# Khrylx/EgoPose

Measured on AMD Instinct MI355X. Metric: env-steps/sec (whole node) ego_mimic PPO, higher is better.
Workload: dtype f64 (rollout kernels K1-K6, physics state) + f32 (policy/value nets)

## Files before the change

egopose_amd/_lib.py:

```python
from __future__ import annotations

import ctypes as C
import os

HERE = os.path.dirname(os.path.abspath(__file__))
LIB_PATH = os.path.join(HERE, "libegopose_hip.so")

EGP_OK = 0
EGP_EXPERT_ROW = 168

c_int_p = C.POINTER(C.c_int32)
c_dbl_p = C.POINTER(C.c_double)
vp = C.c_void_p


class ModelDesc(C.Structure):
    _fields_ = [
        ("nq", C.c_int32), ("nv", C.c_int32), ("nu", C.c_int32), ("nbody", C.c_int32), ("nM", C.c_int32),
        ("body_qpos_start", c_int_p), ("body_ndof", c_int_p), ("dof_parentid", c_int_p), ("dof_Madr", c_int_p),
        ("ee_body", c_int_p),
        ("jkp", c_dbl_p), ("jkd", c_dbl_p), ("a_ref", c_dbl_p), ("a_scale", c_dbl_p), ("torque_lim", c_dbl_p),
        ("b_diffw", c_dbl_p),
        ("sub_dt", C.c_double), ("frame_skip", C.c_int32), ("episode_len", C.c_int32),
        ("w_p", C.c_double), ("w_v", C.c_double), ("w_e", C.c_double), ("w_rp", C.c_double), ("w_rv", C.c_double),
        ("k_p", C.c_double), ("k_v", C.c_double), ("k_e", C.c_double), ("k_rh", C.c_double), ("k_rq", C.c_double),
        ("k_rl", C.c_double), ("k_ra", C.c_double),
        ("v_ord", C.c_double), ("decay", C.c_int32),
        ("obs_heading", C.c_int32), ("obs_keep_root_heading", C.c_int32), ("obs_coord_root", C.c_int32), ("obs_vel", C.c_int32),
        ("action_torque", C.c_int32), ("obs_phase", C.c_int32),
    ]


class ExpertTable(C.Structure):
    _fields_ = [
        ("n_takes", C.c_int32), ("n_frames", C.c_int32), ("take_offset", c_int_p),
        ("qpos", c_dbl_p), ("qvel", c_dbl_p), ("rlinv_local", c_dbl_p), ("rangv", c_dbl_p), ("rq_rmh", c_dbl_p),
        ("ee_pos", c_dbl_p), ("bquat", c_dbl_p), ("bangvel", c_dbl_p), ("head_height_lb", c_dbl_p),
    ]


class SurrogateDesc(C.Structure):
    _fields_ = [
        ("nq", C.c_int32), ("nv", C.c_int32), ("nu", C.c_int32), ("nbody", C.c_int32), ("nM", C.c_int32),
        ("njoint", C.c_int32),
        ("qM0", c_dbl_p), ("Minv0", c_dbl_p), ("body_parent", c_int_p), ("body_pos", c_dbl_p), ("body_ndof", c_int_p),
        ("joint_axis", c_dbl_p), ("joint_anchor", c_dbl_p),
        ("sub_dt", C.c_double), ("damping", C.c_double), ("support_k", C.c_double), ("support_c", C.c_double),
    ]


class DynamicsDesc(C.Structure):
    _fields_ = [("nbody", C.c_int32), ("njoint", C.c_int32), ("body_parent", c_int_p), ("body_pos", c_dbl_p), ("body_com", c_dbl_p),
                ("body_inertia", c_dbl_p), ("body_mass", c_dbl_p), ("body_ndof", c_int_p), ("joint_axis", c_dbl_p),
                ("joint_anchor", c_dbl_p), ("armature", C.c_double), ("gravity", C.c_double * 3)]


class MlpLayer(C.Structure):
    _fields_ = [("wt", vp), ("bias", vp), ("in_dim", C.c_int32), ("out_dim", C.c_int32)]


class GemmDesc(C.Structure):
    _fields_ = [("M", C.c_int32), ("N", C.c_int32), ("K", C.c_int32),
                ("A", vp), ("lda", C.c_int64), ("a_kcontig", C.c_int32),
                ("B", vp), ("ldb", C.c_int64), ("b_kcontig", C.c_int32),
                ("C", vp), ("ldc", C.c_int64),
                ("bias", vp), ("relu", C.c_int32),
                ("mask", vp), ("ldmask", C.c_int64),
                ("terms", C.c_int32), ("splits", C.c_int32), ("accumulate", C.c_int32),
                ("bias_grad", vp), ("workspace", vp),
                ("a_rows", vp), ("A2", vp), ("lda2", C.c_int64), ("a_split", C.c_int32), ("a_src_rows", C.c_int64),
                ("b_krows", vp), ("B2", vp), ("ldb2", C.c_int64), ("b_split", C.c_int32), ("b_src_rows", C.c_int64),
                ("c_rows", vp), ("a_krows", vp)]


class PpoLossDesc(C.Structure):
    _fields_ = [("n", C.c_int32), ("n_pol", C.c_int32), ("act_dim", C.c_int32),
                ("rows", vp), ("pred", vp), ("returns", vp),
                ("mean", vp), ("ld_mean", C.c_int64),
                ("actions", vp), ("ld_act", C.c_int64),
                ("log_std", vp), ("adv", vp),
                ("fixed_logp", vp), ("write_fixed", C.c_int32),
                ("clip_eps", C.c_double), ("inv_n_val", C.c_double), ("inv_n_exp", C.c_double),
                ("d_pred", vp), ("d_mean", vp), ("ld_dmean", C.c_int64), ("d_log_std", vp),
                ("losses", vp), ("workspace", vp)]


class MinibatchPlanDesc(C.Structure):
    _fields_ = [("n", C.c_int32), ("state_dim", C.c_int32), ("act_dim", C.c_int32), ("batch", C.c_int32),
                ("perm", vp),
                ("states", vp), ("ld_states", C.c_int64),
                ("actions", vp), ("ld_act", C.c_int64),
                ("returns", vp), ("adv", vp), ("fixed_logp", vp), ("exps", vp),
                ("out_states", vp), ("out_actions", vp), ("out_returns", vp), ("out_adv", vp), ("out_fixed_logp", vp), ("out_exps", vp),
                ("mb_n_exp", vp)]


class PpoLossMbDesc(C.Structure):
    _fields_ = [("n", C.c_int32), ("act_dim", C.c_int32),
                ("pred", vp), ("returns", vp),
                ("mean", vp), ("ld_mean", C.c_int64),
                ("actions", vp), ("ld_act", C.c_int64),
                ("log_std", vp),
                ("adv", vp), ("fixed_logp", vp), ("exps", vp),
                ("n_exp", vp),
                ("clip_eps", C.c_double),
                ("d_pred", vp),
                ("d_mean", vp), ("ld_dmean", C.c_int64),
                ("d_log_std", vp),
                ("losses", vp)]


PPO_LOSS_MB_MAX_ROWS = 16384


class TcnDesc(C.Structure):
    _fields_ = [("T", C.c_int32), ("B", C.c_int32), ("C_in", C.c_int32), ("C_out", C.c_int32),
                ("taps", C.c_int32), ("shift0", C.c_int32), ("dshift", C.c_int32),
                ("X", vp), ("ldx", C.c_int64),
                ("W", vp),
                ("bias", vp), ("relu", C.c_int32),
                ("mask", vp), ("ldmask", C.c_int64),
                ("gate", vp), ("ldgate", C.c_int64),
                ("X2", vp), ("ldx2", C.c_int64), ("C2", C.c_int32), ("W2", vp), ("b2", vp), ("x2_after_act", C.c_int32),
                ("out", vp), ("ldout", C.c_int64),
                ("out2", vp), ("ldout2", C.c_int64)]


class AdamSegment(C.Structure):
    _fields_ = [("begin", C.c_int64), ("end", C.c_int64),
                ("lr", C.c_double), ("beta1", C.c_double), ("beta2", C.c_double), ("eps", C.c_double), ("weight_decay", C.c_double),
                ("bias1", C.c_double), ("bias2", C.c_double), ("max_norm", C.c_double),
                ("clip_group", C.c_int32)]


ADAM_MAX_SEGMENTS = 8


class RolloutTick(C.Structure):
    _fields_ = [("ctx", vp), ("eng", vp), ("stream", vp),
                ("n_env", C.c_int32), ("nmax", C.c_int32), ("obs_dim", C.c_int32), ("nu", C.c_int32), ("nq", C.c_int32), ("nv", C.c_int32),
                ("ctx_dim", C.c_int32), ("ctx_T", C.c_int32), ("episode_len", C.c_int32), ("reward_job", C.c_int32),
                ("has_fix_head_lb", C.c_int32),
                ("end_reward", C.c_double), ("zf_clip", C.c_double), ("fix_head_lb", C.c_double),
                ("cur_t", vp), ("frame_base", vp), ("e_ind", vp), ("s_ind", vp), ("steps_done", vp),
                ("active", vp), ("active_i32", vp), ("head_z", vp), ("head_lb", vp),
                ("rec_valid", vp), ("rec_done", vp), ("rec_e_ind", vp), ("rec_s_ind", vp),
                ("states", vp), ("next_states", vp), ("actions", vp), ("rewards", vp), ("cinfo", vp),
                ("noise", vp), ("v_out", vp), ("v_stride", C.c_int64),
                ("layers", vp), ("n_layers", C.c_int32), ("activation", C.c_int32), ("log_std", vp),
                ("slab_host", vp), ("slab_dev", vp),
                ("qpos", vp), ("qvel", vp), ("prev_qpos", vp), ("ee", vp),
                ("zf_workspace", vp), ("reset_scratch", vp),
                ("defer_apply", C.c_int32)]


class HostProbeResult(C.Structure):
    _fields_ = [(k, C.c_double) for k in ("pcie_read_gbps", "pcie_read_us_per_pass", "go_rtt_us_p50", "go_rtt_us_p99", "go_rtt_us_max",
                                          "spin_gap_us_max", "spin_gap_us_median_of_thread_max", "spin_lost_frac")] + \
               [(k, C.c_int32) for k in ("pcie_read_rows", "go_rtt_n", "go_in_vram", "large_bar", "spin_threads", "spin_gaps_over_5us")]


class EngineDesc(C.Structure):
    _fields_ = [("n_env", C.c_int32), ("n_threads", C.c_int32), ("n_groups", C.c_int32), ("device_dynamics", C.c_int32)]


PHYS_RESET = C.CFUNCTYPE(C.c_int, vp, C.c_int32, c_dbl_p, c_dbl_p)
PHYS_STEP = C.CFUNCTYPE(C.c_int, vp, C.c_int32, c_dbl_p)
PHYS_DRAIN = C.CFUNCTYPE(C.c_int, vp, C.c_int32, c_dbl_p, c_dbl_p, c_dbl_p, c_dbl_p, c_dbl_p)
PHYS_DESTROY = C.CFUNCTYPE(None, vp)
PHYS_EPOCH = C.CFUNCTYPE(C.c_int64, vp, C.c_int32)


class PhysicsVtable(C.Structure):
    _fields_ = [("user", vp), ("reset", PHYS_RESET), ("step", PHYS_STEP), ("drain", PHYS_DRAIN),
                ("destroy", PHYS_DESTROY), ("name", C.c_char_p), ("inertia_epoch", PHYS_EPOCH)]


_i32, _i64, _f64 = C.c_int32, C.c_int64, C.c_double
SIGNATURES = {
    "egp_last_error": (C.c_char_p, []),
    "egp_version": (C.c_char_p, []),
    "egp_abi_sizeof": (C.c_int64, [C.c_char_p]),
    "egp_obs_dim": (_i32, [vp]),
    "egp_create": (C.c_int, [C.POINTER(ModelDesc), C.c_int, C.POINTER(vp)]),
    "egp_destroy": (C.c_int, [vp]),
    "egp_set_reward_weights": (C.c_int, [vp, C.POINTER(ModelDesc)]),
    "egp_set_pd_variant": (C.c_int, [vp, C.c_int]),
    "egp_upload_experts": (C.c_int, [vp, C.POINTER(ExpertTable)]),
    "egp_reward_simple_f64": (C.c_int, [vp, _i32, vp, vp, vp, vp, C.c_double, _i32, vp, vp, vp]),
    "egp_quat_op_f64": (C.c_int, [_i32, vp, vp, _i32, vp, vp]),
    "egp_quat_op_f32": (C.c_int, [_i32, vp, vp, _i32, vp, vp]),
    "egp_body_quat_f64": (C.c_int, [vp, vp, _i32, vp, vp]),
    "egp_body_quat_f32": (C.c_int, [vp, vp, _i32, vp, vp]),
    "egp_obs_f64": (C.c_int, [vp, vp, vp, vp, _i32, vp, vp]),
    "egp_obs_f32": (C.c_int, [vp, vp, vp, vp, _i32, vp, vp]),
    "egp_pd_torque_f64": (C.c_int, [vp, vp, vp, vp, vp, vp, _i32, vp, vp, vp]),
    "egp_pd_torque_f32": (C.c_int, [vp, vp, vp, vp, vp, vp, _i32, vp, vp, vp]),
    "egp_reward_quat_v3_f64": (C.c_int, [vp, vp, vp, vp, vp, vp, vp, vp, _f64, _i32, vp, vp, vp]),
    "egp_reward_quat_v3_f32": (C.c_int, [vp, vp, vp, vp, vp, vp, vp, vp, _f64, _i32, vp, vp, vp]),
    "egp_pose_features_f64": (C.c_int, [vp, vp, vp, vp, _i32, _i32, vp, vp, vp, vp, vp, vp, vp, vp]),
    "egp_pose_features_f32": (C.c_int, [vp, vp, vp, vp, _i32, _i32, vp, vp, vp, vp, vp, vp, vp, vp]),
    "egp_zfilter_workspace_bytes": (_i64, [_i32, _i32]),
    "egp_zfilter_f64": (C.c_int, [vp, vp, _i32, _i32, vp, vp, _i32, _f64, vp, vp, vp]),
    "egp_zfilter_f32": (C.c_int, [vp, vp, _i32, _i32, vp, vp, _i32, _f64, vp, vp, vp]),
    "egp_obs_zfilter_f64": (C.c_int, [vp, vp, vp, vp, vp, _i32, vp, vp, _f64, vp, vp, _i32, vp, vp]),
    "egp_obs_zfilter_f32": (C.c_int, [vp, vp, vp, vp, vp, _i32, vp, vp, _f64, vp, vp, _i32, vp, vp]),
    "egp_gae_workspace_bytes": (_i64, [_i32]),
    "egp_gae_f64": (C.c_int, [vp, vp, vp, _i32, _f64, _f64, vp, vp, vp, vp, vp]),
    "egp_gae_f32": (C.c_int, [vp, vp, vp, _i32, _f64, _f64, vp, vp, vp, vp, vp]),
    "egp_gae_standardize_f64": (C.c_int, [vp, _i32, vp, vp]),
    "egp_gae_standardize_f32": (C.c_int, [vp, _i32, vp, vp]),
    "egp_lstm_gate_layout": (_i32, []),
    "egp_gather_concat_f32": (C.c_int, [vp, _i64, vp, vp, _i64, _i32, _i32, _i32, vp, _i64, vp]),
    "egp_scatter_rows_f32": (C.c_int, [vp, _i64, vp, _i32, _i32, vp, _i64, vp]),
    "egp_gemm_workspace_floats": (_i64, [_i32, _i32, _i32, _i32]),
    "egp_gemm_f32": (C.c_int, [C.POINTER(GemmDesc), vp]),
    "egp_ppo_loss_workspace_bytes": (_i64, [_i32, _i32, _i32]),
    "egp_ppo_loss_f32": (C.c_int, [C.POINTER(PpoLossDesc), vp]),
    "egp_minibatch_plan_f32": (C.c_int, [C.POINTER(MinibatchPlanDesc), vp]),
    "egp_ppo_loss_mb_f32": (C.c_int, [C.POINTER(PpoLossMbDesc), vp]),
    "egp_tcn_conv_f32": (C.c_int, [C.POINTER(TcnDesc), vp]),
    "egp_adam_workspace_bytes": (_i64, []),
    "egp_adam_step_f32": (C.c_int, [_i32, C.POINTER(AdamSegment), vp, vp, vp, vp, vp, vp, vp]),
    "egp_adam_step_f64": (C.c_int, [_i32, C.POINTER(AdamSegment), vp, vp, vp, vp, vp, vp, vp, vp]),
    "egp_adam_step_f64g": (C.c_int, [_i32, C.POINTER(AdamSegment), vp, vp, vp, vp, vp, vp, vp]),
    "egp_lstm_fwd_f32": (C.c_int, [vp, vp, _i32, _i32, _i32, _i32, vp, vp, vp, vp]),
    "egp_lstm_bwd_f32": (C.c_int, [vp, vp, vp, vp, _i32, _i32, _i32, _i32, vp, vp]),
    "egp_lstm_group_fwd_f32": (C.c_int, [vp, vp, _i32, _i32, _i32, _i32, _i32, C.POINTER(C.c_void_p), _i32, vp, vp, vp]),
    "egp_lstm_group_bwd_f32": (C.c_int, [C.POINTER(C.c_void_p), _i32, vp, vp, vp, _i32, _i32, _i32, _i32, _i32, vp, vp, vp]),
    "egp_rollout_tick_pre": (C.c_int, [vp, _i32, _i32, _i32, _i32, vp, _i32, vp, vp]),
    "egp_rollout_tick_apply": (C.c_int, [vp, _i32, _i32, _i32, _i32, vp, vp]),
    "egp_obs_zfilter_split_max_rows": (C.c_int32, []),
    "egp_obs_zfilter_stats_f64": (C.c_int, [vp, vp, vp, vp, vp, _i32, vp, vp]),
    "egp_obs_zfilter_apply_f64": (C.c_int, [vp, vp, vp, vp, _i32, vp, vp, C.c_double, vp, vp, vp, vp]),
    "egp_policy_gaussian_filter_f32": (C.c_int, [vp, vp, C.c_int64, _i32, vp, vp, vp, vp, _i32, vp, vp, C.c_double, vp, vp, vp,
                                                vp, _i32, _i32, vp, vp, vp, vp, vp, vp, C.c_int64, vp]),
    "egp_rollout_tick_post": (C.c_int, [vp, _i32, _i32, _i32, _i32, vp, vp, vp, vp]),
    "egp_rollout_reset": (C.c_int, [vp, _i32, _i32, _i32, _i32, vp, _i32, vp, vp, vp, vp, vp, vp, vp, vp, vp]),
    "egp_engine_group_stream": (vp, [vp, _i32]),
    "egp_debug_burn": (C.c_int, [C.c_int64, _i32, vp, vp]),
    "egp_lstm_group_fwd_len_f32": (C.c_int, [vp, vp, _i32, _i32, _i32, _i32, _i32, C.POINTER(C.c_void_p), _i32, vp, vp, vp, vp, _i32, vp, vp]),
    "egp_lstm_group_bwd_len_f32": (C.c_int, [C.POINTER(C.c_void_p), _i32, vp, vp, vp, _i32, _i32, _i32, _i32, _i32, vp, vp, vp, vp, _i32, vp]),
    "egp_lstm_group_bwd_rows_f32": (C.c_int, [C.POINTER(C.c_void_p), _i32, vp, vp, vp, _i32, _i32, _i32, _i32, _i32, vp, vp, vp, vp, _i32, vp]),
    "egp_set_dynamics_model": (C.c_int, [vp, C.POINTER(DynamicsDesc)]),
    "egp_dynamics_f64": (C.c_int, [vp, vp, vp, _i32, vp, C.c_int64, vp, vp, vp]),
    "egp_set_pose2d_bodies": (C.c_int, [vp, c_int_p, c_int_p]),
    "egp_pose2d_f64": (C.c_int, [vp, vp, vp, vp, vp, vp, vp, C.c_int64, vp]),
    "egp_mlp_pack_floats": (C.c_int64, [_i32, _i32]),
    "egp_mlp_pack_f32": (C.c_int, [vp, C.c_int64, _i32, _i32, vp, vp]),
    "egp_policy_gaussian_f32": (C.c_int, [vp, C.c_int64, _i32, vp, vp, _i32, _i32, C.POINTER(MlpLayer), _i32, _i32, vp, vp, vp, vp, vp]),
    "egp_policy_forecast_f32": (C.c_int, [vp, C.c_int64, _i32, vp, vp, _i32, C.POINTER(MlpLayer), vp, vp, C.c_int64, _i32,
                                          C.POINTER(MlpLayer), _i32, _i32, vp, vp, vp, vp, vp]),
    "egp_policy_forecast_filter_f32": (C.c_int, [vp, vp, C.c_int64, _i32, vp, vp, vp, vp, _i32, vp, vp, C.c_double, vp, vp, vp,
                                                 C.POINTER(MlpLayer), vp, vp, C.c_int64, C.POINTER(MlpLayer), _i32, _i32, vp, vp, vp, vp, vp]),
    "egp_policy_value_filter_f32": (C.c_int, [vp, vp, C.c_int64, _i32, vp, C.c_int64, _i32, vp, vp, vp, vp, _i32, vp, vp, C.c_double, vp, vp,
                                              C.POINTER(MlpLayer), _i32, _i32, vp, vp, vp, vp, C.POINTER(MlpLayer), _i32, _i32, vp, vp]),
    "egp_policy_gaussian_staged_f32": (C.c_int, [vp, C.c_int64, _i32, vp, vp, _i32, _i32, C.POINTER(MlpLayer), _i32, _i32, vp, vp, vp, vp, vp, vp,
                                                 C.c_int64, vp]),
    "egp_physics_register": (C.c_int, [C.POINTER(PhysicsVtable), _i32, C.POINTER(vp)]),
    "egp_physics_create_surrogate": (C.c_int, [C.POINTER(SurrogateDesc), _i32, C.POINTER(vp)]),
    "egp_physics_destroy": (C.c_int, [vp]),
    "egp_physics_name": (C.c_char_p, [vp]),
    "egp_physics_n_env": (_i32, [vp]),
    "egp_physics_reset_host": (C.c_int, [vp, _i32, vp, vp]),
    "egp_physics_step_host": (C.c_int, [vp, _i32, vp]),
    "egp_physics_drain_host": (C.c_int, [vp, _i32, vp, vp, vp, vp, vp]),
    "egp_engine_create": (C.c_int, [vp, vp, C.POINTER(EngineDesc), C.POINTER(vp)]),
    "egp_engine_destroy": (C.c_int, [vp]),
    "egp_engine_state": (C.c_int, [vp] + [C.POINTER(vp)] * 7),
    "egp_engine_reset": (C.c_int, [vp, vp, _i32, vp, vp, vp]),
    "egp_engine_step_async": (C.c_int, [vp, _i32, vp, vp, vp]),
    "egp_engine_wait": (C.c_int, [vp, _i32, vp]),
    "egp_engine_timing": (C.c_int, [vp, c_dbl_p, c_dbl_p, c_dbl_p, C.POINTER(_i64)]),
    "egp_engine_reset_timing": (C.c_int, [vp]),
    "egp_engine_inertia_uploads": (_i64, [vp]),
    "egp_engine_k1_env_substeps": (_i64, [vp]),
    "egp_engine_event_overhead_ms": (C.c_double, [vp]),
    "egp_engine_set_profile": (C.c_int, [vp, C.c_int]),
    "egp_engine_layout": (C.c_int, [vp, c_int_p, c_int_p, c_int_p, c_int_p]),
    "egp_engine_group_range": (C.c_int, [vp, _i32, c_int_p, c_int_p]),
    "egp_engine_set_reward_job": (C.c_int, [vp, _i32, vp, vp, vp, vp, _f64, vp, vp]),
    "egp_engine_substeps_per_launch": (C.c_int, [vp]),
    "egp_engine_server_trace": (C.c_int, [vp, _i32, vp, vp]),
    "egp_engine_go_words_in_vram": (_i32, [vp]),
    "egp_engine_envs_per_wave": (_i32, [vp, C.POINTER(C.c_int32)]),
    "egp_host_probe": (C.c_int, [_i32, _i32, _i32, C.POINTER(HostProbeResult)]),
    "egp_device_usable_cus": (_i32, [_i32]),
}

_lib = None


class EgpError(RuntimeError):
    pass


def load():
    global _lib
    if _lib is not None:
        return _lib
    if not os.path.exists(LIB_PATH):
        raise EgpError(
            "egopose_amd: %s is missing -- build it with `python -m egopose_amd.build` "
            "(hipcc --offload-arch=gfx950). There is no CPU fallback for the product path." % LIB_PATH)
    lib = C.CDLL(LIB_PATH, mode=C.RTLD_GLOBAL)
    for name, (res, args) in SIGNATURES.items():
        try:
            fn = getattr(lib, name)
        except AttributeError as e:
            raise EgpError("egopose_amd: symbol %s not exported by %s" % (name, LIB_PATH)) from e
        fn.restype = res
        fn.argtypes = args
    _lib = lib
    return lib


def check(rc, what=""):
    if rc == EGP_OK:
        return
    msg = load().egp_last_error().decode("utf-8", "replace")
    text = "%s failed (%d): %s" % (what or "egp call", rc, msg)
    if rc == -1:
        raise ValueError(text)
    raise EgpError(text)


def current_stream(device_index=None):
    import torch
    try:
        if device_index is None:
            device_index = torch._C._cuda_getDevice()
        return C.c_void_p(torch._C._cuda_getCurrentRawStream(device_index))
    except AttributeError:
        return C.c_void_p(torch.cuda.current_stream(device_index).cuda_stream)
```

egopose_amd/csrc/egp_lstm.hip:

```cpp
#include <hip/hip_runtime.h>
#include <math.h>
#include <stdlib.h>

#include "egp_internal.hpp"

namespace egp {

constexpr int KC = 64;

__device__ __forceinline__ float sigmoidf_(float x) { return __builtin_amdgcn_rcpf(1.0f + __expf(-x)); }
__device__ __forceinline__ float tanhf_(float x) { return 2.0f * __builtin_amdgcn_rcpf(1.0f + __expf(-2.0f * x)) - 1.0f; }

typedef float f32x4 __attribute__((ext_vector_type(4)));

#ifndef EGP_LSTM_NT
#define EGP_LSTM_NT 3
#endif
template <typename V> __device__ __forceinline__ void st_save(V *p, V v) {
    if constexpr ((EGP_LSTM_NT & 1) != 0) __builtin_nontemporal_store(v, p); else *p = v;
}
template <typename V> __device__ __forceinline__ V ld_save(const V *p) {
    if constexpr ((EGP_LSTM_NT & 1) != 0) return __builtin_nontemporal_load(p); else return *p;
}
template <typename V> __device__ __forceinline__ void st_dpre(V *p, V v) {
    if constexpr ((EGP_LSTM_NT & 2) != 0) __builtin_nontemporal_store(v, p); else *p = v;
}

struct LstmGroup {
    int ld_g;
    int rev_mask;
    int ld_h;
    int ld_dh;
    long c_stride;
    float *h[4];
    const float *dh[4];
    float *db;
    int db_rows;
    const int *order;
    const int *steps;
    int leave_skipped;
    const int *seq_base;
};

template <int ROWS>
__device__ __forceinline__ int lstm_group_steps(const LstmGroup &grp, int reverse, int r0, int B, int T) {
    if (reverse || !grp.steps) return T;
    int mx = 0;
#pragma unroll
    for (int i = 0; i < ROWS; ++i)
        if (r0 + i < B) mx = max(mx, grp.steps[r0 + i]);
    return min(T, mx);
}

#ifdef EGP_LSTM_TRACE
__device__ long long g_lstm_trace[8];
#define EGP_LT_DECL long long lt_acc[6] = {0, 0, 0, 0, 0, 0}, lt_prev = 0; const bool lt_on = blockIdx.x == EGP_LSTM_TRACE && blockIdx.y == 0 && threadIdx.x == 0
#define EGP_LT_START if (lt_on) lt_prev = (long long)__builtin_readcyclecounter()
#define EGP_LT(i) if (lt_on) { const long long lt_now = (long long)__builtin_readcyclecounter(); lt_acc[i] += lt_now - lt_prev; lt_prev = lt_now; }
#define EGP_LT_END(steps) if (lt_on) { for (int i = 0; i < 6; ++i) g_lstm_trace[i] = lt_acc[i]; g_lstm_trace[6] = (steps); }
#else
#define EGP_LT_DECL do { } while (0)
#define EGP_LT_START do { } while (0)
#define EGP_LT(i) do { } while (0)
#define EGP_LT_END(steps) do { } while (0)
#endif
#ifndef EGP_LSTM_PD1
#define EGP_LSTM_PD1 (NQ == 1 ? 4 : 4)
#endif
#ifndef EGP_LSTM_KCH
#define EGP_LSTM_KCH (NQ == 1 && LH == 64 ? 32 : 64)
#endif
#ifndef EGP_LSTM_BPD
#define EGP_LSTM_BPD ((NQ == 1 && LH == 64) ? 4 : 2)
#endif
#ifndef EGP_LSTM_BKCH
#define EGP_LSTM_BKCH 64
#endif
template <int NQ, int LH, bool FULL, bool TRAIN>
__global__ __launch_bounds__(4 * LH) void k_lstm_fwd_mfma(const float *__restrict__ gx, const float *__restrict__ w_hh, int T, int B,
                                                          LstmGroup grp, float *__restrict__ gates_out, float *__restrict__ c_out) {
    constexpr int LG = 4 * LH, ROWS = 4 * NQ;
    const int prob = (int)(gridDim.y - 1 - blockIdx.y), reverse = (grp.rev_mask >> prob) & 1, ld = grp.ld_g, ld_h = grp.ld_h;
    float *__restrict__ h_out = grp.h[prob];
    gx += prob * LG; w_hh += (long)prob * LG * LH;
    if (TRAIN) { gates_out += prob * LG; c_out += prob * grp.c_stride; }
    constexpr int PD = LH == 128 ? 2 : EGP_LSTM_PD1;
    __shared__ __attribute__((aligned(16))) float s_h[2][ROWS][LH + 4];
    const int lane = threadIdx.x & 63, wave = threadIdx.x >> 6;
    const int u = 16 * wave + (lane >> 2), sub = lane & 3;
    const int r0 = blockIdx.x * ROWS;
    float w[LH];
#pragma unroll
    for (int k = 0; k < LH; ++k) w[k] = w_hh[(long)(sub * LH + u) * LH + k];
    float cst[NQ];
    f32x4 pre[PD][NQ];
    bool live[NQ];
    int rowc[NQ];
#pragma unroll
    for (int q = 0; q < NQ; ++q) {
        cst[q] = 0.f;
        live[q] = FULL || r0 + 4 * q + sub < B;
        const int pos = live[q] ? r0 + 4 * q + sub : B - 1;
        rowc[q] = grp.order ? grp.order[pos] : pos;
    }
    const long gmul = grp.seq_base ? 1 : B;
    long gadd[NQ];
#pragma unroll
    for (int q = 0; q < NQ; ++q) gadd[q] = grp.seq_base ? (long)grp.seq_base[rowc[q]] : (long)rowc[q];
    const int Tp = lstm_group_steps<ROWS>(grp, reverse, r0, B, T);
    for (int i = threadIdx.x; i < 2 * ROWS * (LH + 4); i += 4 * LH) (&s_h[0][0][0])[i] = 0.f;

#define EGP_LSTM_FETCH_GX(STEP, DST)                                                                 \
    {                                                                                                \
        const int f_s = (STEP) < T ? (STEP) : T - 1;                                                 \
        const int f_t = reverse ? T - 1 - f_s : f_s;                                                 \
        _Pragma("unroll") for (int q = 0; q < NQ; ++q)                                               \
            DST[q] = *reinterpret_cast<const f32x4 *>(gx + ((long)f_t * gmul + gadd[q]) * ld + 4 * u); \
    }

    EGP_LT_DECL;
    auto do_step = [&](const int step, const int par, const f32x4 (&init)[NQ]) {
        const int t = reverse ? T - 1 - step : step;
        EGP_LT(0);
        f32x4 acc[NQ], acc2[NQ];
#pragma unroll
        for (int q = 0; q < NQ; ++q) { acc[q] = init[q]; acc2[q] = f32x4{0.f, 0.f, 0.f, 0.f}; }
        constexpr int KCH = EGP_LSTM_KCH;
#pragma unroll
        for (int kc = 0; kc < LH; kc += KCH) {
            float4 hv[NQ][KCH / 4];
#pragma unroll
            for (int q = 0; q < NQ; ++q)
#pragma unroll
                for (int k4 = 0; k4 < KCH / 4; ++k4) hv[q][k4] = *reinterpret_cast<const float4 *>(&s_h[par][4 * q + sub][kc + 4 * k4]);
            __builtin_amdgcn_sched_barrier(0);
            EGP_LT(1);
#pragma unroll
            for (int k4 = 0; k4 < KCH / 4; ++k4)
#pragma unroll
                for (int q = 0; q < NQ; ++q) {
                    acc[q] = __builtin_amdgcn_mfma_f32_4x4x1f32(w[kc + 4 * k4 + 0], hv[q][k4].x, acc[q], 0, 0, 0);
                    acc2[q] = __builtin_amdgcn_mfma_f32_4x4x1f32(w[kc + 4 * k4 + 1], hv[q][k4].y, acc2[q], 0, 0, 0);
                    acc[q] = __builtin_amdgcn_mfma_f32_4x4x1f32(w[kc + 4 * k4 + 2], hv[q][k4].z, acc[q], 0, 0, 0);
                    acc2[q] = __builtin_amdgcn_mfma_f32_4x4x1f32(w[kc + 4 * k4 + 3], hv[q][k4].w, acc2[q], 0, 0, 0);
                }
        }
        EGP_LT(2);
#pragma unroll
        for (int q = 0; q < NQ; ++q) {
            const f32x4 a = acc[q] + acc2[q];
            const float ig = sigmoidf_(a[0]), fg = sigmoidf_(a[1]), gg = tanhf_(a[2]), og = sigmoidf_(a[3]);
            const float cn = fg * cst[q] + ig * gg;
            const float hn = og * tanhf_(cn);
            cst[q] = cn;
            s_h[par ^ 1][4 * q + sub][u] = hn;
            if (FULL || live[q]) {
                const long row = (long)t * B + rowc[q];
                h_out[row * ld_h + u] = hn;
                if (TRAIN) {
                    st_save(reinterpret_cast<f32x4 *>(gates_out + row * ld + 4 * u), f32x4{ig, fg, gg, og});
                    st_save(c_out + row * LH + u, cn);
                }
            }
        }
        EGP_LT(3);
        __syncthreads();
        EGP_LT(4);
    };

#pragma unroll
    for (int d = 0; d < PD; ++d) EGP_LSTM_FETCH_GX(d, pre[d])
    __syncthreads();
    EGP_LT_START;
    int s0 = 0;
    for (; s0 + PD <= Tp; s0 += PD) {
        f32x4 cur[PD][NQ];
#pragma unroll
        for (int d = 0; d < PD; ++d)
#pragma unroll
            for (int q = 0; q < NQ; ++q) cur[d][q] = pre[d][q];
#pragma unroll
        for (int d = 0; d < PD; ++d) EGP_LSTM_FETCH_GX(s0 + PD + d, pre[d])
#pragma unroll
        for (int d = 0; d < PD; ++d) do_step(s0 + d, d & 1, cur[d]);
    }
    for (int d = 0; s0 + d < Tp; ++d) {
        f32x4 last[NQ];
#pragma unroll
        for (int q = 0; q < NQ; ++q) last[q] = d == 0 ? pre[0][q] : d == 1 ? pre[1 % PD][q] : d == 2 ? pre[2 % PD][q] : d == 3 ? pre[3 % PD][q]
                                             : d == 4 ? pre[4 % PD][q] : d == 5 ? pre[5 % PD][q] : pre[6 % PD][q];
        do_step(s0 + d, d & 1, last);
    }
#undef EGP_LSTM_FETCH_GX
    EGP_LT_END(Tp);
    const int Tz = grp.leave_skipped ? lstm_group_steps<8>(grp, reverse, r0 & ~7, B, T) : T;
    for (int t = Tp; t < Tz; ++t)
#pragma unroll
        for (int q = 0; q < NQ; ++q)
            if (FULL || live[q]) h_out[((long)t * B + rowc[q]) * ld_h + u] = 0.f;
}

template <int NQ, int LH, bool FULL>
__global__ __launch_bounds__(4 * LH) void k_lstm_bwd_mfma(const float *__restrict__ gates, const float *__restrict__ cells,
                                                          const float *__restrict__ w_hh, int T, int B, LstmGroup grp,
                                                          float *__restrict__ dpre) {
    constexpr int LG = 4 * LH, NT = 4 * LH, ROWS = 4 * NQ, UH = LH / 64;
    const int prob = (int)(gridDim.y - 1 - blockIdx.y), reverse = (grp.rev_mask >> prob) & 1, ld = grp.ld_g, ld_dh = grp.ld_dh;
    const float *__restrict__ dh_out = grp.dh[prob];
    gates += prob * LG; dpre += prob * LG; cells += prob * grp.c_stride; w_hh += (long)prob * LG * LH;
    constexpr int NP = (ROWS * LH + NT - 1) / NT;
    constexpr int PD = EGP_LSTM_BPD;
    __shared__ __attribute__((aligned(16))) float s_d[ROWS][LG + 4];
    __shared__ float s_part[4][ROWS][LH + 1];
    const int lane = threadIdx.x & 63, wave = threadIdx.x >> 6;
    const int q = wave / UH, uh = wave % UH, sub = lane & 3;
    const int r0 = blockIdx.x * ROWS;
    float w[LH];
#pragma unroll
    for (int cc = 0; cc < LH; ++cc) {
        const int n = q * LH + cc;
        w[cc] = w_hh[(long)((n & 3) * LH + (n >> 2)) * LH + 64 * uh + lane];
    }
    float dc_next[NP], dh_rec[NP];
    f32x4 dsum[NP];
    f32x4 pg[PD][NP];
    float pc[PD][NP], pdh[PD][NP];
    bool live[NP];
    int rowc[NP];
#pragma unroll
    for (int qq = 0; qq < NP; ++qq) {
        dc_next[qq] = 0.f; dh_rec[qq] = 0.f; dsum[qq] = f32x4{0.f, 0.f, 0.f, 0.f};
        const int r = (threadIdx.x + NT * qq) / LH;
        live[qq] = FULL || r0 + r < B;
        const int pos = live[qq] ? r0 + r : B - 1;
        rowc[qq] = grp.order ? grp.order[pos] : pos;
    }
    const int Tp = lstm_group_steps<ROWS>(grp, reverse, r0, B, T);
    const int Tz = grp.leave_skipped ? lstm_group_steps<8>(grp, reverse, r0 & ~7, B, T) : T;
    for (int t = Tp; t < Tz; ++t)
#pragma unroll
        for (int qq = 0; qq < NP; ++qq)
            if (FULL || live[qq])
                *reinterpret_cast<f32x4 *>(dpre + ((long)t * B + rowc[qq]) * ld + 4 * ((threadIdx.x + NT * qq) % LH)) = f32x4{0.f, 0.f, 0.f, 0.f};

#define EGP_LSTM_FETCH(STEP, D)                                                                      \
    {                                                                                                \
        const int f_s = (STEP) > 0 ? (STEP) : 0;                                                     \
        const int f_t = reverse ? T - 1 - f_s : f_s;                                                 \
        _Pragma("unroll") for (int qq = 0; qq < NP; ++qq) {                                          \
            const int j = (threadIdx.x + NT * qq) % LH;                                              \
            const long row = (long)f_t * B + rowc[qq];                                               \
            pg[D][qq] = ld_save(reinterpret_cast<const f32x4 *>(gates + row * ld + 4 * j));         \
            pc[D][qq] = ld_save(cells + row * LH + j);                                               \
            pdh[D][qq] = dh_out[row * ld_dh + j];                                                    \
        }                                                                                            \
    }

    auto do_step = [&](const int step, const f32x4 (&g4)[NP], const float (&cc_)[NP], const float (&cdh)[NP], const float (&cprev)[NP]) {
        const int t = reverse ? T - 1 - step : step;
#pragma unroll
        for (int qq = 0; qq < NP; ++qq) {
            const int p = threadIdx.x + NT * qq, r = p / LH, j = p % LH;
            const float ig = g4[qq][0], fg = g4[qq][1], gg = g4[qq][2], og = g4[qq][3];
            const float c_prev = step > 0 ? cprev[qq] : 0.f;
            const float tc = tanhf_(cc_[qq]);
            const float dh = (FULL || live[qq] ? cdh[qq] : 0.f) + dh_rec[qq];
            const float dc = dh * og * (1.f - tc * tc) + dc_next[qq];
            const float d_o = dh * tc * og * (1.f - og);
            const float di = dc * gg * ig * (1.f - ig);
            const float df = dc * c_prev * fg * (1.f - fg);
            const float dg = dc * ig * (1.f - gg * gg);
            dc_next[qq] = dc * fg;
            const f32x4 d4 = f32x4{di, df, dg, d_o};
            if (FULL || live[qq]) { st_dpre(reinterpret_cast<f32x4 *>(dpre + ((long)t * B + rowc[qq]) * ld + 4 * j), d4); dsum[qq] += d4; }
            *reinterpret_cast<f32x4 *>(&s_d[r][4 * j]) = d4;
        }
        __syncthreads();
        f32x4 acc[NQ], acc2[NQ];
#pragma unroll
        for (int qd = 0; qd < NQ; ++qd) acc[qd] = acc2[qd] = f32x4{0.f, 0.f, 0.f, 0.f};
#pragma unroll
        for (int kc = 0; kc < LH; kc += EGP_LSTM_BKCH) {
            float4 dv[NQ][EGP_LSTM_BKCH / 4];
#pragma unroll
            for (int qd = 0; qd < NQ; ++qd)
#pragma unroll
                for (int c4 = 0; c4 < EGP_LSTM_BKCH / 4; ++c4) dv[qd][c4] = *reinterpret_cast<const float4 *>(&s_d[4 * qd + sub][q * LH + kc + 4 * c4]);
            __builtin_amdgcn_sched_barrier(0);
#pragma unroll
            for (int c4 = 0; c4 < EGP_LSTM_BKCH / 4; ++c4)
#pragma unroll
                for (int qd = 0; qd < NQ; ++qd) {
                    acc[qd] = __builtin_amdgcn_mfma_f32_4x4x1f32(w[kc + 4 * c4 + 0], dv[qd][c4].x, acc[qd], 0, 0, 0);
                    acc2[qd] = __builtin_amdgcn_mfma_f32_4x4x1f32(w[kc + 4 * c4 + 1], dv[qd][c4].y, acc2[qd], 0, 0, 0);
                    acc[qd] = __builtin_amdgcn_mfma_f32_4x4x1f32(w[kc + 4 * c4 + 2], dv[qd][c4].z, acc[qd], 0, 0, 0);
                    acc2[qd] = __builtin_amdgcn_mfma_f32_4x4x1f32(w[kc + 4 * c4 + 3], dv[qd][c4].w, acc2[qd], 0, 0, 0);
                }
        }
#pragma unroll
        for (int qd = 0; qd < NQ; ++qd) {
            const f32x4 a = acc[qd] + acc2[qd];
#pragma unroll
            for (int i = 0; i < 4; ++i) s_part[q][4 * qd + sub][64 * uh + (lane & ~3) + i] = a[i];
        }
        __syncthreads();
#pragma unroll
        for (int qq = 0; qq < NP; ++qq) {
            const int p = threadIdx.x + NT * qq, r = p / LH, j = p % LH;
            dh_rec[qq] = s_part[0][r][j] + s_part[1][r][j] + s_part[2][r][j] + s_part[3][r][j];
        }
    };

#pragma unroll
    for (int d = 0; d < PD; ++d) EGP_LSTM_FETCH(Tp - 1 - d, d)
    int s0 = Tp - 1;
    for (; s0 - PD + 1 >= 0; s0 -= PD) {
        f32x4 cg[PD][NP];
        float cc_[PD][NP], cdh[PD][NP];
#pragma unroll
        for (int d = 0; d < PD; ++d)
#pragma unroll
            for (int qq = 0; qq < NP; ++qq) {
                cg[d][qq] = pg[d][qq];
                cc_[d][qq] = pc[d][qq];
                cdh[d][qq] = pdh[d][qq];
            }
#pragma unroll
        for (int d = 0; d < PD; ++d) EGP_LSTM_FETCH(s0 - PD - d, d)
#pragma unroll
        for (int d = 0; d < PD; ++d)
            do_step(s0 - d, cg[d], cc_[d], cdh[d], d + 1 < PD ? cc_[d + 1 < PD ? d + 1 : 0] : pc[0]);
    }
#pragma unroll
    for (int d = 0; d < PD - 1; ++d)
        if (s0 - d >= 0) do_step(s0 - d, pg[d], pc[d], pdh[d], pc[d + 1]);
#undef EGP_LSTM_FETCH
    if (grp.db) {
        __syncthreads();
#pragma unroll
        for (int qq = 0; qq < NP; ++qq) {
            const int p = threadIdx.x + NT * qq;
            *reinterpret_cast<f32x4 *>(&s_d[p / LH][4 * (p % LH)]) = dsum[qq];
        }
        __syncthreads();
        if (grp.db_rows) {
            for (int p = threadIdx.x; p < ROWS * LG; p += NT) {
                const int r = p / LG, c = p % LG;
                if (FULL || r0 + r < B) grp.db[((long)prob * B + r0 + r) * LG + c] = s_d[r][c];
            }
        } else {
            for (int c = threadIdx.x; c < LG; c += NT) {
                float a = 0.f;
#pragma unroll
                for (int r = 0; r < ROWS; ++r) a += s_d[r][c];
                atomicAdd(grp.db + prob * LG + c, a);
            }
        }
    }
}

}

using namespace egp;

static int lstm_quads(int B) { return B >= 4096 ? 2 : 1; }

static int lstm_launch_check(const char *what) {
    hipError_t e = hipGetLastError();
    if (e != hipSuccess) {
        set_error("launch of %s failed: %s", what, hipGetErrorString(e));
        return EGP_E_HIP;
    }
    return EGP_OK;
}

template <int NQ, int LH>
static void launch_fwd_mfma_t(bool full, bool train, int P, const float *gx, const float *w_hh, int T, int B, const LstmGroup &g,
                              float *gates_save, float *cells_save, hipStream_t s) {
    const dim3 grid((B + 4 * NQ - 1) / (4 * NQ), P), block(4 * LH);
    if (full && train) k_lstm_fwd_mfma<NQ, LH, true, true><<<grid, block, 0, s>>>(gx, w_hh, T, B, g, gates_save, cells_save);
    else if (full) k_lstm_fwd_mfma<NQ, LH, true, false><<<grid, block, 0, s>>>(gx, w_hh, T, B, g, gates_save, cells_save);
    else if (train) k_lstm_fwd_mfma<NQ, LH, false, true><<<grid, block, 0, s>>>(gx, w_hh, T, B, g, gates_save, cells_save);
    else k_lstm_fwd_mfma<NQ, LH, false, false><<<grid, block, 0, s>>>(gx, w_hh, T, B, g, gates_save, cells_save);
}
static void launch_fwd_mfma(int hidden, int P, const float *gx, const float *w_hh, int T, int B, const LstmGroup &g,
                            float *gates_save, float *cells_save, hipStream_t s) {
    const int nq = hidden == 64 ? lstm_quads(B) : 1;
    const bool full = B % (4 * nq) == 0, train = gates_save != nullptr;
    if (hidden == 128) launch_fwd_mfma_t<1, 128>(full, train, P, gx, w_hh, T, B, g, gates_save, cells_save, s);
    else if (nq >= 2) launch_fwd_mfma_t<2, 64>(full, train, P, gx, w_hh, T, B, g, gates_save, cells_save, s);
    else launch_fwd_mfma_t<1, 64>(full, train, P, gx, w_hh, T, B, g, gates_save, cells_save, s);
}

template <int NQ, int LH>
static void launch_bwd_mfma_t(bool full, int P, const float *gates_save, const float *cells_save, const float *w_hh, int T, int B,
                              const LstmGroup &g, float *d_pre, hipStream_t s) {
    const dim3 grid((B + 4 * NQ - 1) / (4 * NQ), P), block(4 * LH);
    if (full) k_lstm_bwd_mfma<NQ, LH, true><<<grid, block, 0, s>>>(gates_save, cells_save, w_hh, T, B, g, d_pre);
    else k_lstm_bwd_mfma<NQ, LH, false><<<grid, block, 0, s>>>(gates_save, cells_save, w_hh, T, B, g, d_pre);
}
static void launch_bwd_mfma(int hidden, int P, const float *gates_save, const float *cells_save, const float *w_hh, int T, int B,
                            const LstmGroup &g, float *d_pre, hipStream_t s) {
    const int nq = hidden == 64 ? lstm_quads(B) : 1;
    const bool full = B % (4 * nq) == 0;
    if (hidden == 128) launch_bwd_mfma_t<1, 128>(full, P, gates_save, cells_save, w_hh, T, B, g, d_pre, s);
    else if (nq >= 2) launch_bwd_mfma_t<2, 64>(full, P, gates_save, cells_save, w_hh, T, B, g, d_pre, s);
    else launch_bwd_mfma_t<1, 64>(full, P, gates_save, cells_save, w_hh, T, B, g, d_pre, s);
}

static int lstm_group_bwd(const float *const *dh_out, int32_t ld_dh, const float *gates_save, const float *cells_save, const float *w_hh,
                          int32_t T, int32_t B, int32_t hidden, int32_t n_problems, int32_t reverse_mask, float *d_pre, float *d_bias,
                          int db_rows, const int32_t *seq_order, const int32_t *seq_steps, int32_t leave_skipped, void *stream) {
    EGP_REQUIRE((seq_order == nullptr) == (seq_steps == nullptr), "seq_order and seq_steps go together");
    EGP_REQUIRE(hidden == 64 || hidden == 128, "egp_lstm kernels are built for hidden size 64 and 128");
    EGP_REQUIRE(n_problems >= 1 && n_problems <= 4, "1..4 problems per group");
    EGP_REQUIRE(T >= 0 && B >= 0, "negative size");
    if (T == 0 || B == 0) return EGP_OK;
    EGP_REQUIRE(dh_out && gates_save && cells_save && w_hh && d_pre && ld_dh >= hidden, "NULL pointer / d h_out row stride below the hidden size");
    LstmGroup g = {};
    g.ld_g = 4 * hidden * n_problems; g.rev_mask = reverse_mask; g.ld_dh = ld_dh; g.c_stride = (long)T * B * hidden; g.db = d_bias; g.db_rows = db_rows;
    for (int p = 0; p < n_problems; ++p) {
        EGP_REQUIRE(dh_out[p], "NULL d h_out");
        g.dh[p] = dh_out[p];
    }
    g.order = seq_order; g.steps = seq_steps; g.leave_skipped = seq_steps && leave_skipped;
    launch_bwd_mfma(hidden, n_problems, gates_save, cells_save, w_hh, T, B, g, d_pre, (hipStream_t)stream);
    return lstm_launch_check("k_lstm_bwd_mfma (group)");
}

extern "C" {

int32_t egp_lstm_gate_layout(void) { return EGP_LSTM_GATES_UNIT_MAJOR; }

int egp_lstm_fwd_f32(const float *gates_x, const float *w_hh, int32_t T, int32_t B, int32_t hidden, int32_t reverse,
                     float *h_out, float *gates_save, float *cells_save, void *stream) {
    EGP_REQUIRE(hidden == 64 || hidden == 128, "egp_lstm kernels are built for hidden size 64 and 128");
    EGP_REQUIRE(T >= 0 && B >= 0, "negative size");
    if (T == 0 || B == 0) return EGP_OK;
    EGP_REQUIRE(gates_x && w_hh && h_out, "NULL pointer");
    EGP_REQUIRE((gates_save == nullptr) == (cells_save == nullptr), "gates_save and cells_save go together");
    hipStream_t s = (hipStream_t)stream;
    LstmGroup g = {};
    g.ld_g = 4 * hidden; g.rev_mask = reverse ? 1 : 0; g.ld_h = hidden; g.h[0] = h_out;
    launch_fwd_mfma(hidden, 1, gates_x, w_hh, T, B, g, gates_save, cells_save, s);
    return lstm_launch_check("k_lstm_fwd");
}

int egp_lstm_bwd_f32(const float *dh_out, const float *gates_save, const float *cells_save, const float *w_hh, int32_t T, int32_t B,
                     int32_t hidden, int32_t reverse, float *d_pre, void *stream) {
    EGP_REQUIRE(hidden == 64 || hidden == 128, "egp_lstm kernels are built for hidden size 64 and 128");
    EGP_REQUIRE(T >= 0 && B >= 0, "negative size");
    if (T == 0 || B == 0) return EGP_OK;
    EGP_REQUIRE(dh_out && gates_save && cells_save && w_hh && d_pre, "NULL pointer");
    hipStream_t s = (hipStream_t)stream;
    LstmGroup g = {};
    g.ld_g = 4 * hidden; g.rev_mask = reverse ? 1 : 0; g.ld_dh = hidden; g.dh[0] = dh_out;
    launch_bwd_mfma(hidden, 1, gates_save, cells_save, w_hh, T, B, g, d_pre, s);
    return lstm_launch_check("k_lstm_bwd");
}

int egp_lstm_group_fwd_f32(const float *gates_x, const float *w_hh, int32_t T, int32_t B, int32_t hidden, int32_t n_problems,
                           int32_t reverse_mask, float *const *h_out, int32_t ld_h, float *gates_save, float *cells_save, void *stream) {
    return egp_lstm_group_fwd_len_f32(gates_x, w_hh, T, B, hidden, n_problems, reverse_mask, h_out, ld_h, gates_save, cells_save, nullptr, nullptr, 0,
                                      nullptr, stream);
}

int egp_lstm_group_fwd_len_f32(const float *gates_x, const float *w_hh, int32_t T, int32_t B, int32_t hidden, int32_t n_problems,
                               int32_t reverse_mask, float *const *h_out, int32_t ld_h, float *gates_save, float *cells_save,
                               const int32_t *seq_order, const int32_t *seq_steps, int32_t leave_skipped, const int32_t *seq_base,
                               void *stream) {
    EGP_REQUIRE((seq_order == nullptr) == (seq_steps == nullptr), "seq_order and seq_steps go together");
    EGP_REQUIRE(!seq_base || !gates_save || gates_save != gates_x, "a frame table cannot double as the saved gates (rows are shared between sequences)");
    EGP_REQUIRE(hidden == 64 || hidden == 128, "egp_lstm kernels are built for hidden size 64 and 128");
    EGP_REQUIRE(n_problems >= 1 && n_problems <= 4, "1..4 problems per group");
    EGP_REQUIRE(T >= 0 && B >= 0, "negative size");
    if (T == 0 || B == 0) return EGP_OK;
    EGP_REQUIRE(gates_x && w_hh && h_out && ld_h >= hidden, "NULL pointer / h_out row stride below the hidden size");
    EGP_REQUIRE((gates_save == nullptr) == (cells_save == nullptr), "gates_save and cells_save go together");
    LstmGroup g = {};
    g.ld_g = 4 * hidden * n_problems; g.rev_mask = reverse_mask; g.ld_h = ld_h; g.c_stride = (long)T * B * hidden;
    for (int p = 0; p < n_problems; ++p) {
        EGP_REQUIRE(h_out[p], "NULL h_out");
        g.h[p] = h_out[p];
    }
    g.order = seq_order; g.steps = seq_steps; g.leave_skipped = seq_steps && leave_skipped; g.seq_base = seq_base;
    launch_fwd_mfma(hidden, n_problems, gates_x, w_hh, T, B, g, gates_save, cells_save, (hipStream_t)stream);
    return lstm_launch_check("k_lstm_fwd_mfma (group)");
}

int egp_lstm_group_bwd_f32(const float *const *dh_out, int32_t ld_dh, const float *gates_save, const float *cells_save, const float *w_hh,
                           int32_t T, int32_t B, int32_t hidden, int32_t n_problems, int32_t reverse_mask, float *d_pre, float *d_bias,
                           void *stream) {
    return egp_lstm_group_bwd_len_f32(dh_out, ld_dh, gates_save, cells_save, w_hh, T, B, hidden, n_problems, reverse_mask, d_pre, d_bias, nullptr,
                                      nullptr, 0, stream);
}

int egp_lstm_group_bwd_len_f32(const float *const *dh_out, int32_t ld_dh, const float *gates_save, const float *cells_save, const float *w_hh,
                               int32_t T, int32_t B, int32_t hidden, int32_t n_problems, int32_t reverse_mask, float *d_pre, float *d_bias,
                               const int32_t *seq_order, const int32_t *seq_steps, int32_t leave_skipped, void *stream) {
    return lstm_group_bwd(dh_out, ld_dh, gates_save, cells_save, w_hh, T, B, hidden, n_problems, reverse_mask, d_pre, d_bias, 0, seq_order,
                          seq_steps, leave_skipped, stream);
}

int egp_lstm_group_bwd_rows_f32(const float *const *dh_out, int32_t ld_dh, const float *gates_save, const float *cells_save, const float *w_hh,
                                int32_t T, int32_t B, int32_t hidden, int32_t n_problems, int32_t reverse_mask, float *d_pre, float *d_bias_rows,
                                const int32_t *seq_order, const int32_t *seq_steps, int32_t leave_skipped, void *stream) {
    EGP_REQUIRE(d_bias_rows, "NULL d_bias_rows");
    if (T == 0 && B > 0 && n_problems >= 1 && n_problems <= 4) {
        EGP_HIP_CHECK(hipMemsetAsync(d_bias_rows, 0, sizeof(float) * (size_t)n_problems * B * 4 * hidden, (hipStream_t)stream));
        return EGP_OK;
    }
    return lstm_group_bwd(dh_out, ld_dh, gates_save, cells_save, w_hh, T, B, hidden, n_problems, reverse_mask, d_pre, d_bias_rows, 1, seq_order,
                          seq_steps, leave_skipped, stream);
}

}
```

egopose_amd/gemm.py:

```python
from __future__ import annotations

import ctypes as C
import os

import torch

from . import _lib as L

_WS = {}


def enabled():
    return os.environ.get("EGP_GEMM", "hip") != "torch"


def default_terms():
    t = os.environ.get("EGP_GEMM_TERMS", "6")
    if t not in ("1", "3", "6"):
        raise ValueError("EGP_GEMM_TERMS must be 1, 3 or 6, got %r" % t)
    return int(t)


_WS_MAX = 8


def _workspace(n_floats, device):
    key = (str(device), int(torch.cuda.current_stream(device).cuda_stream))
    buf = _WS.pop(key, None)
    if buf is None or buf.numel() < n_floats:
        buf = torch.empty(max(int(n_floats), 1 << 20), dtype=torch.float32, device=device)
    _WS[key] = buf
    while len(_WS) > _WS_MAX:
        _WS.pop(next(iter(_WS)))
    return buf


def _mat(t, name):
    if not (t.is_cuda and t.dtype == torch.float32 and t.dim() == 2):
        raise ValueError("%s must be a 2-D float32 HIP tensor, got %s %s" % (name, tuple(t.shape), t.dtype))
    if t.shape[1] > 1 and t.stride(1) != 1:
        raise ValueError("%s must have unit stride along its second dimension (strides %s)" % (name, t.stride()))
    return t


def _ld(t):
    return t.stride(0) if t.shape[0] > 1 else max(t.shape[1], 1)


_CUS = {}


def usable_cus(device=None):
    if not torch.cuda.is_available():
        return 256
    dev = torch.cuda.current_device() if device is None else int(device)
    if dev not in _CUS:
        n = int(L.load().egp_device_usable_cus(dev))
        _CUS[dev] = n if n > 0 else 256
    return _CUS[dev]


def pick_splits(M, n_out, K):
    cus = usable_cus()
    if M == 1:
        return max(1, min(cus, K // 128))
    tiles = ((M + 127) // 128) * ((n_out + 127) // 128)
    return max(1, min(cus // tiles, K // 256))


def _index(t, name):
    if not (t.is_cuda and t.dtype == torch.int64 and t.dim() == 1 and t.is_contiguous()):
        raise ValueError("%s must be a contiguous 1-D int64 HIP tensor" % name)
    return t


def gemm(A, B, a_kcontig=True, b_kcontig=True, bias=None, relu=False, mask=None, terms=None, splits=1, want_bias_grad=False,
         out=None, bias_grad_out=None, accumulate=False, a_rows=None, a2=None, b_krows=None, b2=None, c_rows=None, a_krows=None):
    A, B = _mat(A, "A"), _mat(B, "B")
    if accumulate and not (splits > 1 or want_bias_grad):
        raise ValueError("accumulate goes with splits > 1 or want_bias_grad (a plain product overwrites `out`)")
    M, K = (A.shape if a_kcontig else A.shape[::-1])
    N, Kb = (B.shape if b_kcontig else B.shape[::-1])
    a_split = b_split = 0
    if a_rows is not None or a2 is not None:
        if not a_kcontig:
            raise ValueError("a_rows / a2 go with a k-contiguous A")
        if a_rows is not None:
            M = _index(a_rows, "a_rows").shape[0]
        if a2 is not None:
            _mat(a2, "a2")
            if a2.shape[0] != M:
                raise ValueError("a2 has %d rows, the operand %d" % (a2.shape[0], M))
            a_split, K = K, K + a2.shape[1]
    if a_krows is not None:
        if a_kcontig:
            raise ValueError("a_krows goes with A given as (K, M)")
        K = _index(a_krows, "a_krows").shape[0]
    if b_krows is not None or b2 is not None:
        if b_kcontig:
            raise ValueError("b_krows / b2 go with B given as (K, N)")
        if b_krows is not None:
            Kb = _index(b_krows, "b_krows").shape[0]
        if b2 is not None:
            _mat(b2, "b2")
            if b2.shape[0] != Kb:
                raise ValueError("b2 has %d rows, the operand %d" % (b2.shape[0], Kb))
            b_split, N = N, N + b2.shape[1]
    if K != Kb:
        raise ValueError("inner dimensions differ: %d vs %d" % (K, Kb))
    dev = A.device
    if c_rows is not None:
        if out is None or _index(c_rows, "c_rows").shape[0] != M:
            raise ValueError("c_rows needs `out` (the scatter destination) and one entry per result row")
    elif out is None:
        out = torch.empty(M, N, dtype=torch.float32, device=dev)
    _mat(out, "out")
    d = L.GemmDesc()
    d.M, d.N, d.K = M, N, K
    if a_rows is not None:
        d.a_rows, d.a_src_rows = a_rows.data_ptr(), A.shape[0]
    if a2 is not None:
        d.A2, d.lda2, d.a_split = a2.data_ptr(), _ld(a2), a_split
    if b_krows is not None:
        d.b_krows, d.b_src_rows = b_krows.data_ptr(), B.shape[0]
    if b2 is not None:
        d.B2, d.ldb2, d.b_split = b2.data_ptr(), _ld(b2), b_split
    if c_rows is not None:
        d.c_rows = c_rows.data_ptr()
    if a_krows is not None:
        d.a_krows = a_krows.data_ptr()
    d.A, d.lda, d.a_kcontig = A.data_ptr(), _ld(A), 1 if a_kcontig else 0
    d.B, d.ldb, d.b_kcontig = B.data_ptr(), _ld(B), 1 if b_kcontig else 0
    d.C, d.ldc = out.data_ptr(), _ld(out)
    d.bias = bias.data_ptr() if bias is not None else None
    d.relu = 1 if relu else 0
    if mask is not None:
        _mat(mask, "mask")
        d.mask, d.ldmask = mask.data_ptr(), _ld(mask)
    d.terms = int(terms or default_terms())
    d.splits = int(splits)
    d.accumulate = 1 if accumulate else 0
    bg = None
    if want_bias_grad:
        bg = bias_grad_out if bias_grad_out is not None else torch.empty(M, dtype=torch.float32, device=dev)
        d.bias_grad = bg.data_ptr()
    if splits > 1 or want_bias_grad:
        ws = _workspace(L.load().egp_gemm_workspace_floats(M, N, 1 if want_bias_grad else 0, int(splits)), dev)
        d.workspace = ws.data_ptr()
    L.check(L.load().egp_gemm_f32(C.byref(d), L.current_stream()), "egp_gemm_f32")
    return (out, bg) if want_bias_grad else out


def linear_fwd(x, W, b=None, relu=False, terms=None):
    return gemm(x, W, True, True, bias=b, relu=relu, terms=terms)


def linear_dgrad(dy, W, mask=None, n_cols=None, terms=None):
    Wv = W if n_cols is None else W[:, :n_cols]
    return gemm(dy, Wv, True, False, mask=mask, terms=terms)


def linear_wgrad(dy, x, want_bias=True, terms=None):
    K, M = dy.shape
    n_out = x.shape[1] + (1 if want_bias else 0)
    return gemm(dy, x, False, False, terms=terms, splits=pick_splits(M, n_out, K), want_bias_grad=want_bias)


class MlpHead(torch.autograd.Function):

    @staticmethod
    def forward(ctx, x, n_grad_cols, *params):
        Ws, bs = params[0::2], params[1::2]
        hs = [x.contiguous()]
        for i, (W, b) in enumerate(zip(Ws, bs)):
            hs.append(linear_fwd(hs[-1], W.contiguous(), b, relu=i < len(Ws) - 1))
        ctx.save_for_backward(*hs[:-1], *Ws)
        ctx.n_layers, ctx.n_grad_cols = len(Ws), int(n_grad_cols)
        return hs[-1]

    @staticmethod
    def backward(ctx, dout):
        nl = ctx.n_layers
        hs, Ws = ctx.saved_tensors[:nl], ctx.saved_tensors[nl:]
        dz = dout.contiguous()
        grads = [None] * (2 * nl)
        dx = None
        for i in range(nl - 1, -1, -1):
            need_w, need_b = ctx.needs_input_grad[2 + 2 * i], ctx.needs_input_grad[3 + 2 * i]
            if need_w or need_b:
                dW, db = linear_wgrad(dz, hs[i], want_bias=True)
                grads[2 * i], grads[2 * i + 1] = (dW if need_w else None), (db if need_b else None)
            if i > 0:
                dz = linear_dgrad(dz, Ws[i].contiguous(), mask=hs[i])
            elif ctx.needs_input_grad[0]:
                nc = ctx.n_grad_cols
                W0 = Ws[0].contiguous()
                if nc >= W0.shape[1]:
                    dx = linear_dgrad(dz, W0)
                else:
                    dx = torch.zeros(dz.shape[0], W0.shape[1], dtype=dz.dtype, device=dz.device)
                    gemm(dz, W0[:, :nc], True, False, out=dx[:, :nc])
        return (dx, None, *grads)


def mlp_head_available(x, layers, head, activation):
    if isinstance(x, GatheredInput):
        x = x.x
    if not (enabled() and x.is_cuda and x.dtype == torch.float32 and x.dim() == 2 and activation is torch.relu):
        return False
    return all(l.weight.dtype == torch.float32 and l.bias is not None and l.weight.is_cuda for l in list(layers) + [head])


def mlp_head(x, layers, head, n_grad_cols=None):
    params = []
    for l in list(layers) + [head]:
        params += [l.weight, l.bias]
    nc = x.shape[1] if n_grad_cols is None else int(n_grad_cols)
    return MlpHead.apply(x, nc, *params)


class GatheredInput:

    def __init__(self, ctx2d, idx, x):
        self.ctx2d, self.idx, self.x = ctx2d, idx, x
        self.shape = (x.shape[0], ctx2d.shape[1] + x.shape[1])
        self.dtype, self.device, self.is_cuda = x.dtype, x.device, x.is_cuda

    def dim(self):
        return 2

    def size(self, k=None):
        return torch.Size(self.shape) if k is None else self.shape[k]

    def materialize(self):
        return GatherConcat.apply(self.ctx2d, self.idx, self.x)

    def __getitem__(self, ind):
        if torch.is_tensor(ind) and ind.dtype == torch.int64 and ind.dim() == 1:
            return GatheredInput(self.ctx2d, self.idx.index_select(0, ind), self.x.index_select(0, ind))
        return self.materialize()[ind]


def fused_gather_available(H, n_hidden, S):
    import os
    return enabled() and default_terms() == 6 and os.environ.get("EGP_GEMM_WS", "1") != "0" and H % 128 == 0 and n_hidden % 4 == 0 \
        and S >= 32


def fused_rows_available():
    import os
    return enabled() and default_terms() == 6 and os.environ.get("EGP_GEMM_WS", "1") != "0"


class GatherMlpHead(torch.autograd.Function):

    @staticmethod
    def forward(ctx, ctx2d, idx, x, *params):
        Ws, bs = params[0::2], params[1::2]
        ctx2d, x = ctx2d.contiguous(), (x if x.stride(1) == 1 else x.contiguous())
        h = gemm(ctx2d, Ws[0].contiguous(), True, True, bias=bs[0], relu=len(Ws) > 1, a_rows=idx, a2=x)
        hs = [h]
        for i in range(1, len(Ws)):
            hs.append(linear_fwd(hs[-1], Ws[i].contiguous(), bs[i], relu=i < len(Ws) - 1))
        ctx.save_for_backward(ctx2d, idx, x, *hs[:-1], *Ws)
        ctx.n_layers = len(Ws)
        return hs[-1]

    @staticmethod
    def backward(ctx, dout):
        nl = ctx.n_layers
        ctx2d, idx, x = ctx.saved_tensors[:3]
        hs, Ws = ctx.saved_tensors[3:3 + nl - 1], ctx.saved_tensors[3 + nl - 1:]
        dz = dout.contiguous()
        grads = [None] * (2 * nl)
        for i in range(nl - 1, 0, -1):
            need_w, need_b = ctx.needs_input_grad[3 + 2 * i], ctx.needs_input_grad[4 + 2 * i]
            if need_w or need_b:
                dW, db = linear_wgrad(dz, hs[i - 1], want_bias=True)
                grads[2 * i], grads[2 * i + 1] = (dW if need_w else None), (db if need_b else None)
            dz = linear_dgrad(dz, Ws[i].contiguous(), mask=hs[i - 1])
        H, S = ctx2d.shape[1], x.shape[1]
        if ctx.needs_input_grad[3] or ctx.needs_input_grad[4]:
            n = dz.shape[0]
            dW, db = gemm(dz, ctx2d, False, False, splits=pick_splits(dz.shape[1], H + S + 1, n), want_bias_grad=True, b_krows=idx, b2=x)
            grads[0], grads[1] = (dW if ctx.needs_input_grad[3] else None), (db if ctx.needs_input_grad[4] else None)
        dctx = None
        if ctx.needs_input_grad[0]:
            dctx = torch.zeros_like(ctx2d)
            gemm(dz, Ws[0][:, :H], True, False, out=dctx, c_rows=idx)
        return (dctx, None, None, *grads)


def gather_mlp_head(gi, layers, head):
    params = []
    for l in list(layers) + [head]:
        params += [l.weight, l.bias]
    return GatherMlpHead.apply(gi.ctx2d, gi.idx, gi.x, *params)


class GatherConcat(torch.autograd.Function):

    @staticmethod
    def forward(ctx, ctx2d, idx, x):
        n, H, S = idx.shape[0], ctx2d.shape[1], x.shape[1]
        out = torch.empty(n, H + S, dtype=torch.float32, device=x.device)
        L.check(L.load().egp_gather_concat_f32(ctx2d.data_ptr(), _ld(ctx2d), idx.data_ptr(), x.data_ptr(), _ld(x), n, H, S,
                                               out.data_ptr(), H + S, L.current_stream()), "egp_gather_concat_f32")
        ctx.save_for_backward(idx)
        ctx.shape = tuple(ctx2d.shape)
        return out

    @staticmethod
    def backward(ctx, dout):
        (idx,) = ctx.saved_tensors
        if not ctx.needs_input_grad[0]:
            return None, None, None
        R, H = ctx.shape
        dout = _mat(dout if dout.stride(1) == 1 else dout.contiguous(), "dout")
        dctx = torch.zeros(R, H, dtype=torch.float32, device=dout.device)
        L.check(L.load().egp_scatter_rows_f32(dout.data_ptr(), _ld(dout), idx.data_ptr(), idx.shape[0], H, dctx.data_ptr(), H,
                                              L.current_stream()), "egp_scatter_rows_f32")
        return dctx, None, None


def gather_concat_available(ctx2d, idx, x):
    return (enabled() and x.is_cuda and ctx2d.dtype == torch.float32 and x.dtype == torch.float32 and ctx2d.dim() == 2 and x.dim() == 2
            and ctx2d.is_contiguous() and x.stride(1) == 1 and idx.dtype == torch.int64 and idx.is_contiguous() and not x.requires_grad)
```

egopose_amd/lstm.py:

```python
from __future__ import annotations

import ctypes as C
import os

import numpy as np
import torch

from . import _lib as L
from . import gemm as G

HIDDEN_SIZES = (64, 128)


def available(x, cell):
    return (x.is_cuda and x.dtype == torch.float32 and cell.hidden_size in HIDDEN_SIZES
            and cell.weight_hh.dtype == torch.float32 and cell.bias_ih is not None)


def _s():
    return L.current_stream()


def _p(t):
    return C.c_void_p(t.data_ptr()) if t is not None else C.c_void_p(0)


_PERM = {}


def _gate_perm(hidden, device):
    if L.load().egp_lstm_gate_layout() == 0:
        return None
    key = (hidden, str(device))
    if key not in _PERM:
        n = torch.arange(4 * hidden, device=device)
        perm = (n % 4) * hidden + n // 4
        _PERM[key] = (perm, torch.argsort(perm))
    return _PERM[key]


def _stacked_perm(hidden, P, device):
    key = (hidden, P, str(device))
    if key not in _PERM:
        perm, inv = _gate_perm(hidden, device)
        off = (torch.arange(P, device=device) * 4 * hidden).unsqueeze(1)
        _PERM[key] = ((perm.unsqueeze(0) + off).reshape(-1), (inv.unsqueeze(0) + off).reshape(-1))
    return _PERM[key]


class LstmDirection(torch.autograd.Function):

    @staticmethod
    def forward(ctx, x, w_ih, w_hh, b_ih, b_hh, reverse, train):
        lib = L.load()
        T, B, D = x.shape
        HIDDEN = w_hh.shape[1]
        x2 = x.reshape(T * B, D)
        pp = _gate_perm(HIDDEN, x.device)
        bias = b_ih + b_hh
        w_in = w_ih
        if pp is not None:
            w_in, bias = w_ih.index_select(0, pp[0]), bias.index_select(0, pp[0])
        if G.enabled():
            gx = G.linear_fwd(x2, w_in.contiguous(), bias).view(T, B, 4 * HIDDEN)
        else:
            gx = torch.addmm(bias, x2, w_in.t()).view(T, B, 4 * HIDDEN)
        h_buf = torch.empty(T + 1, B, HIDDEN, dtype=x.dtype, device=x.device)
        h_buf[T if reverse else 0].zero_()
        h = h_buf[:T] if reverse else h_buf[1:]
        cells = torch.empty(T, B, HIDDEN, dtype=x.dtype, device=x.device) if train else None
        w_hh_c = w_hh.contiguous()
        L.check(lib.egp_lstm_fwd_f32(_p(gx), _p(w_hh_c), T, B, HIDDEN, 1 if reverse else 0, _p(h),
                                     _p(gx if train else None), _p(cells), _s()), "egp_lstm_fwd_f32")
        if train:
            ctx.save_for_backward(x2, w_in, w_hh_c, h_buf, gx, cells)
            ctx.reverse = bool(reverse)
            ctx.shape = (T, B, D)
        return h

    @staticmethod
    def backward(ctx, dh):
        lib = L.load()
        x2, w_in, w_hh, h_buf, gates, cells = ctx.saved_tensors
        T, B, D = ctx.shape
        HIDDEN = w_hh.shape[1]
        h = h_buf
        dpre = torch.empty(T, B, 4 * HIDDEN, dtype=h.dtype, device=h.device)
        L.check(lib.egp_lstm_bwd_f32(_p(dh.contiguous()), _p(gates), _p(cells), _p(w_hh), T, B, HIDDEN,
                                     1 if ctx.reverse else 0, _p(dpre), _s()), "egp_lstm_bwd_f32")
        h_prev = h_buf[1:] if ctx.reverse else h_buf[:T]
        pp = _gate_perm(HIDDEN, h.device)
        if G.enabled():
            d2 = dpre.view(T * B, 4 * HIDDEN)
            dw_ih, dbias = G.linear_wgrad(d2, x2, want_bias=True)
            dw_hh = G.linear_wgrad(d2, h_prev.reshape(T * B, HIDDEN), want_bias=False)
            if pp is not None:
                dw_ih, dw_hh, dbias = dw_ih.index_select(0, pp[1]), dw_hh.index_select(0, pp[1]), dbias.index_select(0, pp[1])
            d_w_ih = dw_ih if ctx.needs_input_grad[1] else None
            d_w_hh = dw_hh if ctx.needs_input_grad[2] else None
            d_b = dbias if (ctx.needs_input_grad[3] or ctx.needs_input_grad[4]) else None
        else:
            xh1 = torch.cat((x2.view(T, B, D), h_prev, h.new_ones(T, B, 1)), 2)
            dw = torch.bmm(dpre.transpose(1, 2), xh1).sum(0)
            if pp is not None:
                dw = dw.index_select(0, pp[1])
            d_w_ih = dw[:, :D].contiguous() if ctx.needs_input_grad[1] else None
            d_w_hh = dw[:, D:D + HIDDEN].contiguous() if ctx.needs_input_grad[2] else None
            d_b = dw[:, D + HIDDEN].contiguous() if (ctx.needs_input_grad[3] or ctx.needs_input_grad[4]) else None
        d_x = dpre.view(T * B, 4 * HIDDEN).mm(w_in).view(T, B, D) if ctx.needs_input_grad[0] else None
        return d_x, d_w_ih, d_w_hh, d_b, d_b, None, None


class LstmGroup(torch.autograd.Function):

    @staticmethod
    def forward(ctx, x, reverse_mask, P, width, train, ragged, frames, *params):
        lib = L.load()
        T, B, D = x.shape
        w_ih, w_hh, b_ih, b_hh = params[0::4], params[1::4], params[2::4], params[3::4]
        H = w_hh[0].shape[1]
        perm, inv = _gate_perm(H, x.device)
        x2 = x.reshape(T * B, D)
        pord = [p for p in range(P) if not (reverse_mask >> p) & 1] + [p for p in range(P) if (reverse_mask >> p) & 1]
        nf = sum(1 for p in range(P) if not (reverse_mask >> p) & 1)
        kmask = sum(1 << q for q in range(nf, P))
        bperm, _ = _stacked_perm(H, P, x.device)
        w_in = torch.cat([w_ih[p] for p in pord], 0).index_select(0, bperm)
        bias = (torch.cat([b_ih[p] for p in pord]) + torch.cat([b_hh[p] for p in pord])).index_select(0, bperm)
        rows = None
        if ragged is not None and ragged.rows is not None and 0 < nf and G.enabled() and G.fused_rows_available() \
                and ragged.T == T and ragged.rows.shape[0] >= 4096 and D >= 32:
            rows = ragged.rows
        seq_base, gates_buf = None, None
        if frames is not None and G.enabled():
            table, seq_base = frames
            gx = G.linear_fwd(table, w_in, bias)
            gates_buf = torch.empty(T * B, P * 4 * H, dtype=x.dtype, device=x.device) if train else None
        elif rows is not None:
            gx = torch.empty(T * B, P * 4 * H, dtype=x.dtype, device=x.device)
            nfc = nf * 4 * H
            G.gemm(x2, w_in[:nfc], True, True, bias=bias[:nfc], a_rows=rows, c_rows=rows, out=gx[:, :nfc])
            if nf < P:
                G.gemm(x2, w_in[nfc:], True, True, bias=bias[nfc:], out=gx[:, nfc:])
        elif G.enabled():
            gx = G.linear_fwd(x2, w_in, bias)
        else:
            gx = torch.addmm(bias, x2, w_in.t())
        w_hh_all = torch.stack([w_hh[p].contiguous() for p in pord], 0)
        n_out, W = P // width, width * H
        h_buf = torch.empty(n_out, T + 2, B, W, dtype=x.dtype, device=x.device)
        h_buf[:, 0].zero_()
        h_buf[:, T + 1].zero_()
        cells = torch.empty(P, T, B, H, dtype=x.dtype, device=x.device) if train else None
        base, esz = h_buf.data_ptr(), h_buf.element_size()
        ptrs = (C.c_void_p * P)(*[base + esz * (((p // width) * (T + 2) + 1) * B * W + (p % width) * H) for p in pord])
        order, steps = (ragged.order, ragged.steps) if ragged is not None else (None, None)
        leave = int(rows is not None and train)
        gates = gates_buf if seq_base is not None else (gx if train else None)
        L.check(lib.egp_lstm_group_fwd_len_f32(_p(gx), _p(w_hh_all), T, B, H, P, kmask, ptrs, W,
                                               _p(gates), _p(cells), _p(order), _p(steps), leave, _p(seq_base), _s()), "egp_lstm_group_fwd_len_f32")
        outs = tuple(h_buf[i, 1:T + 1] for i in range(n_out))
        if train:
            ctx.save_for_backward(x2, w_in, w_hh_all, h_buf, gates, cells)
            ctx.meta = (T, B, D, H, P, width, reverse_mask)
            ctx.ragged, ctx.rows, ctx.pord, ctx.nf, ctx.kmask, ctx.leave = ragged, rows, pord, nf, kmask, leave
        return outs

    @staticmethod
    def backward(ctx, *douts):
        lib = L.load()
        x2, w_in, w_hh_all, h_buf, gates, cells = ctx.saved_tensors
        T, B, D, H, P, width, reverse_mask = ctx.meta
        W = width * H
        perm, inv = _gate_perm(H, x2.device)
        douts = [d.contiguous() if d is not None else h_buf.new_zeros(T, B, W) for d in douts]
        ragged, rows, pord, nf, kmask = ctx.ragged, ctx.rows, ctx.pord, ctx.nf, ctx.kmask
        esz = h_buf.element_size()
        ptrs = (C.c_void_p * P)(*[douts[p // width].data_ptr() + esz * (p % width) * H for p in pord])
        dpre = torch.empty(T * B, P * 4 * H, dtype=x2.dtype, device=x2.device)
        db_rows = torch.empty(P, B, 4 * H, dtype=x2.dtype, device=x2.device)
        order, steps = (ragged.order, ragged.steps) if ragged is not None else (None, None)
        leave = int(bool(ctx.leave) and not ctx.needs_input_grad[0])
        L.check(lib.egp_lstm_group_bwd_rows_f32(ptrs, W, _p(gates), _p(cells), _p(w_hh_all), T, B, H, P, kmask, _p(dpre), _p(db_rows),
                                                _p(order), _p(steps), leave, _s()), "egp_lstm_group_bwd_rows_f32")
        db = db_rows.sum(1)
        d3 = dpre.view(T, B, P * 4 * H)
        use_g = G.enabled()
        nfc = nf * 4 * H
        if rows is not None:
            n_rows = rows.shape[0]
            parts = [G.gemm(dpre[:, :nfc], x2, False, False, splits=G.pick_splits(nfc, D, n_rows), a_krows=rows, b_krows=rows)]
            if nf < P:
                parts.append(G.linear_wgrad(dpre[:, nfc:], x2, want_bias=False))
            dw_ih_all = torch.cat(parts, 0)
        elif use_g:
            dw_ih_all = G.linear_wgrad(dpre, x2, want_bias=False)
        else:
            dw_ih_all = torch.bmm(d3.transpose(1, 2), x2.view(T, B, D)).sum(0)
        grads = [None] * (4 * P)
        _, binv = _stacked_perm(H, P, x2.device)
        dw_ih_t = dw_ih_all.index_select(0, binv)
        db_t = db.reshape(-1).index_select(0, binv).view(P, 4 * H)
        for q, p in enumerate(pord):
            rev = (kmask >> q) & 1
            slab = h_buf[p // width, 2:] if rev else h_buf[p // width, :T]
            h_prev = slab[:, :, (p % width) * H:(p % width + 1) * H]
            if use_g:
                dq, hq = dpre[:, q * 4 * H:(q + 1) * 4 * H], slab.reshape(T * B, W)[:, (p % width) * H:(p % width + 1) * H]
                if rows is not None and not rev:
                    dw_hh = G.gemm(dq, hq, False, False, splits=G.pick_splits(4 * H, H, rows.shape[0]), a_krows=rows, b_krows=rows).index_select(0, inv)
                else:
                    dw_hh = G.linear_wgrad(dq, hq, want_bias=False).index_select(0, inv)
            else:
                dw_hh = torch.bmm(d3[:, :, q * 4 * H:(q + 1) * 4 * H].transpose(1, 2), h_prev).sum(0).index_select(0, inv)
            dw_ih = dw_ih_t[q * 4 * H:(q + 1) * 4 * H]
            d_b = db_t[q]
            grads[4 * p:4 * p + 4] = [dw_ih, dw_hh, d_b, d_b]
        d_x = dpre.mm(w_in).view(T, B, D) if ctx.needs_input_grad[0] else None
        return (d_x, None, None, None, None, None, None, *grads)


def _wants_grad(x, params):
    return torch.is_grad_enabled() and (x.requires_grad or any(p.requires_grad for p in params))


def group_available(x, cells):
    if not cells or len(cells) > 4 or L.load().egp_lstm_gate_layout() == 0:
        return False
    c0 = cells[0]
    return all(available(x, c) and c.hidden_size == c0.hidden_size and c.input_size == c0.input_size for c in cells)


class Ragged:

    def __init__(self, order, steps, rows, n_seq, T):
        self.order, self.steps, self.rows, self.n_seq, self.T = order, steps, rows, n_seq, T


def ragged_order(seq_steps, device, T=None):
    st = np.asarray(torch.as_tensor(seq_steps).cpu().numpy(), dtype=np.int64).reshape(-1)
    B = st.shape[0]
    order = np.argsort(-st, kind="stable")
    st_sorted = st[order]
    rows = None
    if T is not None and B > 0:
        wg = np.maximum.reduceat(st_sorted, np.arange(0, B, 8))
        t_wg = np.minimum(np.repeat(wg, 8)[:B], int(T))
        n = int(t_wg.sum())
        if n < 0.9 * T * B:
            t_seq = np.empty(B, np.int64)
            t_seq[order] = t_wg
            stepped = np.arange(int(T), dtype=np.int64)[:, None] < t_seq[None, :]
            rows = torch.as_tensor(np.flatnonzero(stepped), dtype=torch.int64, device=device)
    return Ragged(torch.as_tensor(order, dtype=torch.int32, device=device), torch.as_tensor(st_sorted, dtype=torch.int32, device=device),
                  rows, B, T)


def lstm_group(x, cells, reverses, pairs=False, ragged=None, frames=None):
    mask = sum(1 << i for i, r in enumerate(reverses) if r)
    params = [t for c in cells for t in (c.weight_ih, c.weight_hh, c.bias_ih, c.bias_hh)]
    if ragged is not None and ragged.n_seq != x.shape[1]:
        ragged = None
    if frames is not None:
        table, base = frames
        ok = (table.is_cuda and table.dtype == x.dtype and table.dim() == 2 and table.shape[1] == x.shape[2] and table.is_contiguous()
              and base.dtype == torch.int32 and base.is_cuda and base.is_contiguous() and base.shape[0] == x.shape[1] and not x.requires_grad)
        if not ok:
            frames = None
    return list(LstmGroup.apply(x.contiguous(), mask, len(cells), 2 if pairs else 1, _wants_grad(x, params), ragged, frames, *params))


def lstm_direction(cell, x, reverse):
    params = (cell.weight_ih, cell.weight_hh, cell.bias_ih, cell.bias_hh)
    return LstmDirection.apply(x, *params, bool(reverse), _wants_grad(x, params))
```

egopose_amd/nets.py:

```python
from __future__ import annotations

import math

import numpy as np
import torch
import torch.nn as nn

import os

from . import dist as _dist
from . import gemm as _gemm
from . import gemm_tuning as _tuning
from . import lstm as _hip_lstm
from . import tcn as _tcn
from .tcn import TemporalConvNet

_FWD_BUCKETS = 1
_LSTM_IMPL = os.environ.get("EGP_LSTM", "hip")

_ACT = {"tanh": torch.tanh, "relu": torch.relu, "sigmoid": torch.sigmoid}


def bucket_rows(x):
    if _tuning.enabled() and x.is_cuda and x.dim() == 2 and x.shape[0] >= 4 * _tuning.ROW_BUCKET:
        pad = _tuning.pad_to(x.shape[0], _tuning.ROW_BUCKET)
        if pad:
            return nn.functional.pad(x, (0, 0, 0, pad)), x.shape[0]
    return x, None


def _take_lengths(take_offset, n_rows):
    off = np.asarray(take_offset, dtype=np.int64).ravel()
    return np.diff(np.concatenate((off, [int(n_rows)])))


def _check_windows(take_len, expert_ind, start_ind, before, after):
    e = np.asarray(expert_ind, dtype=np.int64).ravel()
    s = np.asarray(start_ind, dtype=np.int64).ravel()
    if e.size == 0:
        return
    if e.min() < 0 or e.max() >= len(take_len):
        raise ValueError("take index out of range: [%d, %d] with %d takes" % (e.min(), e.max(), len(take_len)))
    bad = (s - before < 0) | (s + after > take_len[e])
    if bad.any():
        k = int(np.nonzero(bad)[0][0])
        raise ValueError("CNN-feature window [%d, %d) leaves take %d (%d frames): %d of %d windows do"
                         % (s[k] - before, s[k] + after, e[k], take_len[e[k]], int(bad.sum()), e.size))


class MLP(nn.Module):
    def __init__(self, input_dim, hidden_dims=(128, 128), activation="tanh"):
        super().__init__()
        self.activation = _ACT[activation]
        dims = [input_dim] + list(hidden_dims)
        self.out_dim = dims[-1]
        self.affine_layers = nn.ModuleList(nn.Linear(a, b) for a, b in zip(dims[:-1], dims[1:]))

    def forward(self, x):
        for layer in self.affine_layers:
            x = self.activation(layer(x))
        return x


class _DiagLogProb(torch.autograd.Function):

    @staticmethod
    def forward(ctx, value, loc, log_std):
        inv_std = torch.exp(-log_std)
        z = (value - loc) * inv_std
        ctx.save_for_backward(z, inv_std)
        const = log_std.sum() + 0.5 * log_std.shape[-1] * math.log(2.0 * math.pi)
        return (z * z).sum(1, keepdim=True).mul_(-0.5).sub_(const)

    @staticmethod
    def backward(ctx, g):
        z, inv_std = ctx.saved_tensors
        d_loc = d_ls = None
        if ctx.needs_input_grad[1]:
            d_loc = (z * inv_std).mul_(g)
        if ctx.needs_input_grad[2]:
            d_ls = ((z * z - 1.0) * g).sum(0, keepdim=True)
        d_val = None
        if ctx.needs_input_grad[0]:
            d_val = -((z * inv_std) * g)
        return d_val, d_loc, d_ls


class DiagGaussian(torch.distributions.Normal):

    def __init__(self, loc, scale, log_std_row=None):
        super().__init__(loc, scale, validate_args=False)
        self._log_std_row = log_std_row

    def kl(self):
        mu0, s0 = self.loc.detach(), self.scale.detach()
        ls1 = self.scale.log()
        out = ls1 - ls1.detach() + (s0.pow(2) + (mu0 - self.loc).pow(2)) / (2.0 * self.scale.pow(2)) - 0.5
        return out.sum(1, keepdim=True)

    def log_prob(self, value):
        if self._log_std_row is not None and value.dim() == 2:
            return _DiagLogProb.apply(value, self.loc, self._log_std_row)
        return super().log_prob(value).sum(1, keepdim=True)

    def mean_sample(self):
        return self.loc


class Policy(nn.Module):
    def select_action(self, x, mean_action=False):
        dist = self.forward(x)
        return dist.mean_sample() if mean_action else dist.sample()

    def get_kl(self, x):
        return self.forward(x).kl()

    def get_log_prob(self, x, action):
        return self.forward(x).log_prob(action)


class PolicyGaussian(Policy):
    def __init__(self, net, action_dim, net_out_dim=None, log_std=0, fix_std=False):
        super().__init__()
        self.type = "gaussian"
        self.net = net
        self.action_mean = nn.Linear(net.out_dim if net_out_dim is None else net_out_dim, action_dim)
        with torch.no_grad():
            self.action_mean.weight.mul_(0.1)
            self.action_mean.bias.zero_()
        self.action_log_std = nn.Parameter(torch.full((1, action_dim), float(log_std)), requires_grad=not fix_std)

    def mean_std(self, x):
        if _gemm.mlp_head_available(x, getattr(self.net, "affine_layers", ()), self.action_mean, getattr(self.net, "activation", None)):
            if isinstance(x, _gemm.GatheredInput):
                mean = _gemm.gather_mlp_head(x, self.net.affine_layers, self.action_mean)
            else:
                mean = _gemm.mlp_head(x, self.net.affine_layers, self.action_mean, getattr(x, "_egp_ctx_cols", None))
        else:
            if isinstance(x, _gemm.GatheredInput):
                x = x.materialize()
            x, n = bucket_rows(x)
            mean = self.action_mean(self.net(x))
            if n is not None:
                mean = mean[:n]
        return mean, torch.exp(self.action_log_std).expand_as(mean)

    def forward(self, x):
        mean, std = self.mean_std(x)
        return DiagGaussian(mean, std, self.action_log_std if self.action_log_std.dim() == 2 and self.action_log_std.shape[0] == 1 else None)

    def get_fim(self, x):
        mean, _ = self.mean_std(x)
        cov_inv = self.action_log_std.exp().pow(-2).squeeze(0).repeat(x.size(0))
        offset, std_id, std_index = 0, 0, 0
        for i, (name, p) in enumerate(self.named_parameters()):
            if name == "action_log_std":
                std_id, std_index = i, offset
            offset += p.numel()
        return cov_inv.detach(), mean, {"std_id": std_id, "std_index": std_index}


class Value(nn.Module):
    def __init__(self, net, net_out_dim=None):
        super().__init__()
        self.net = net
        self.value_head = nn.Linear(net.out_dim if net_out_dim is None else net_out_dim, 1)
        with torch.no_grad():
            self.value_head.weight.mul_(0.1)
            self.value_head.bias.zero_()

    def forward(self, x):
        if _gemm.mlp_head_available(x, getattr(self.net, "affine_layers", ()), self.value_head, getattr(self.net, "activation", None)):
            if isinstance(x, _gemm.GatheredInput):
                return _gemm.gather_mlp_head(x, self.net.affine_layers, self.value_head)
            return _gemm.mlp_head(x, self.net.affine_layers, self.value_head, getattr(x, "_egp_ctx_cols", None))
        if isinstance(x, _gemm.GatheredInput):
            x = x.materialize()
        x, n = bucket_rows(x)
        out = self.value_head(self.net(x))
        return out if n is None else out[:n]


def _lstm_sweep(cell: nn.LSTMCell, x, reverse):
    T, B, _ = x.shape
    H = cell.hidden_size
    if _LSTM_IMPL != "torch" and _hip_lstm.available(x, cell):
        return _hip_lstm.lstm_direction(cell, x.contiguous(), reverse)
    fused_ok = x.is_cuda and x.dtype in (torch.float32, torch.float16, torch.bfloat16)
    if fused_ok:
        h0 = x.new_zeros(1, B, H)
        xs = x.flip(0) if reverse else x
        out, _, _ = torch._VF.lstm(xs, (h0, h0), [cell.weight_ih, cell.weight_hh, cell.bias_ih, cell.bias_hh],
                                   True, 1, 0.0, cell.training, False, False)
        return out.flip(0) if reverse else out
    gates_x = torch.addmm(cell.bias_ih + cell.bias_hh, x.reshape(T * B, -1), cell.weight_ih.t()).view(T, B, 4 * H)
    w_hh_t = cell.weight_hh.t()
    h = x.new_zeros(B, H)
    c = x.new_zeros(B, H)
    outs = [None] * T
    for t in (range(T - 1, -1, -1) if reverse else range(T)):
        g = torch.addmm(gates_x[t], h, w_hh_t)
        i, f, gg, o = g.chunk(4, dim=1)
        c = torch.sigmoid(f) * c + torch.sigmoid(i) * torch.tanh(gg)
        h = torch.sigmoid(o) * torch.tanh(c)
        outs[t] = h
    return torch.stack(outs, 0)


class RNN(nn.Module):
    def __init__(self, input_dim, out_dim, cell_type="lstm", bi_dir=False):
        super().__init__()
        self.input_dim, self.out_dim, self.cell_type, self.bi_dir = input_dim, out_dim, cell_type, bi_dir
        self.mode = "batch"
        make = nn.LSTMCell if cell_type == "lstm" else nn.GRUCell
        hidden = out_dim // 2 if bi_dir else out_dim
        self.rnn_f = make(input_dim, hidden)
        if bi_dir:
            self.rnn_b = make(input_dim, hidden)
        self.hx = self.cx = None
        self.ragged = None

    def set_mode(self, mode):
        self.mode = mode

    def initialize(self, batch_size=1):
        if self.mode == "step":
            p = self.rnn_f.weight_hh
            self.hx = p.new_zeros(batch_size, self.rnn_f.hidden_size)
            self.cx = p.new_zeros(batch_size, self.rnn_f.hidden_size) if self.cell_type == "lstm" else None

    def _sweep(self, cell, x, reverse):
        if self.cell_type == "lstm":
            return _lstm_sweep(cell, x, reverse)
        h = x.new_zeros(x.size(1), cell.hidden_size)
        outs = [None] * x.size(0)
        for t in (range(x.size(0) - 1, -1, -1) if reverse else range(x.size(0))):
            h = cell(x[t], h)
            outs[t] = h
        return torch.stack(outs, 0)

    def forward(self, x):
        if self.mode == "step":
            self.hx = self.hx.to(x.device)
            if self.cell_type == "lstm":
                self.hx, self.cx = self.rnn_f(x, (self.hx, self.cx.to(x.device)))
            else:
                self.hx = self.rnn_f(x, self.hx)
            return self.hx
        if (self.bi_dir and self.cell_type == "lstm" and _LSTM_IMPL != "torch"
                and _hip_lstm.group_available(x, [self.rnn_f, self.rnn_b])):
            return _hip_lstm.lstm_group(x, [self.rnn_f, self.rnn_b], [False, True], pairs=True, ragged=self.ragged)[0]
        out = self._sweep(self.rnn_f, x, False)
        if self.bi_dir:
            out = torch.cat((out, self._sweep(self.rnn_b, x, True)), 2)
        return out


def _video_net(input_dim, v_hdim, v_net_type, v_net_param, causal):
    if v_net_type == "lstm":
        return RNN(input_dim, v_hdim, v_net_type, bi_dir=not causal)
    if v_net_type == "tcn":
        return _tcn.from_param(input_dim, v_hdim, v_net_param, causal)
    raise ValueError("v_net_type must be 'lstm' or 'tcn', got %r" % (v_net_type,))


def _run_video_net(v_net, x):
    return v_net.forward_tm(x) if isinstance(v_net, _tcn.TemporalConvNet) else v_net(x)


class VideoStateNet(nn.Module):

    def __init__(self, cnn_feat_dim, v_hdim=128, v_margin=10, v_net_type="lstm", v_net_param=None, causal=False):
        super().__init__()
        self.mode = "test"
        self.cnn_feat_dim, self.v_hdim, self.v_margin, self.v_net_type = cnn_feat_dim, v_hdim, v_margin, v_net_type
        self.v_net = _video_net(cnn_feat_dim, v_hdim, v_net_type, v_net_param, causal)
        self.v_out = None
        self.t = 0
        self.indices = None
        self.gather_indices = None
        self._gather_tm = None
        self._gather_unique = False
        self.cnn_feat_ctx = None
        self._buckets = None
        self._v_ctx = None
        self._ctx_key = None
        self._cnn_table = None
        self._ragged = None

    def set_mode(self, mode):
        self.mode = mode

    def forward_v_net(self, x):
        return _run_video_net(self.v_net, x)

    def attach_feature_table(self, table, take_offset):
        host = np.asarray(take_offset, dtype=np.int64)
        cur = getattr(self, "_cnn_table", None)
        if cur is not None and cur[0] is table and np.array_equal(getattr(self, "_take_offset_host", None), host):
            return
        self._cnn_table = (table, torch.as_tensor(host, dtype=torch.long, device=table.device))
        self._take_offset_host = host.copy()
        self._take_len = _take_lengths(take_offset, table.shape[0])

    def check_windows(self, expert_ind, start_ind, length):
        _check_windows(self._take_len, expert_ind, start_ind, self.v_margin, length + self.v_margin)

    def window_features(self, expert_ind, start_ind, length):
        table, off = self._cnn_table
        m = self.v_margin
        base = off[expert_ind.long()] + start_ind.long() - m
        rows = base.unsqueeze(0) + torch.arange(length + 2 * m, device=table.device).unsqueeze(1)
        return table[rows]

    def initialize(self, x):
        m = self.v_margin
        if self.mode == "test":
            p = next(self.parameters())
            x = x.to(device=p.device, dtype=p.dtype)
            single = x.dim() == 2
            out = self.forward_v_net(x.unsqueeze(1) if single else x)[m:-m]
            self.v_out = out.squeeze(1) if single else out
            self.t = 0
            return
        masks, cnn_feat, v_metas = x
        device, dtype = masks.device, masks.dtype
        self._frames = None
        ends = torch.nonzero(masks == 0).flatten().cpu().numpy()
        n = masks.shape[0]
        starts = np.concatenate(([0], ends[:-1] + 1))
        lens = ends - starts + 1
        max_len = _dist.global_max(int(lens.max()), device)
        idx = np.arange(n)
        ep_of = np.repeat(np.arange(len(ends)), lens)
        covered = int(ends[-1]) + 1
        idx[:covered] = ep_of * max_len + (np.arange(covered) - np.repeat(starts, lens))
        self.indices = idx
        meta = np.asarray(v_metas)[ends]
        if self._cnn_table is not None and self._cnn_table[0].device == device:
            pad = _tuning.pad_to(len(ends), _tuning.EPISODE_BUCKET) if _tuning.enabled() and len(ends) >= 4 * _tuning.EPISODE_BUCKET else 0
            if pad:
                meta = np.concatenate((meta, np.repeat(meta[:1], pad, axis=0)), 0)
            self.check_windows(meta[:, 0], meta[:, 1], max_len)
            e_ind = torch.as_tensor(meta[:, 0], device=device)
            s_ind = torch.as_tensor(meta[:, 1], device=device)
            self.cnn_feat_ctx = self.window_features(e_ind, s_ind, max_len).to(dtype)
            table = self._cnn_table[0]
            n_rows = self.cnn_feat_ctx.shape[0] * self.cnn_feat_ctx.shape[1]
            if table.dtype == dtype and table.is_contiguous() and 2 * table.shape[0] <= n_rows:
                base = self._take_offset_host[meta[:, 0].astype(np.int64)] + meta[:, 1].astype(np.int64) - m
                self._frames = (table, torch.as_tensor(base.astype(np.int32), device=device))
        else:
            ctx = np.zeros((max_len + 2 * m, len(ends), self.cnn_feat_dim))
            for e, (ei, si) in enumerate(meta):
                ctx[:, e, :] = cnn_feat[int(ei)][int(si) - m: int(si) + max_len + m]
            self.cnn_feat_ctx = torch.as_tensor(ctx, dtype=dtype, device=device)
        self.gather_indices = torch.as_tensor(idx, dtype=torch.long, device=device)
        tm = ((idx % max_len) + m) * self.cnn_feat_ctx.shape[1] + idx // max_len
        self._gather_tm = torch.as_tensor(tm, dtype=torch.long, device=device)
        self._gather_unique = covered == n or np.unique(tm).size == tm.size
        self._ctx_key = (int(max_len), meta.shape[0], hash(meta.tobytes()))
        steps = np.zeros(self.cnn_feat_ctx.shape[1], np.int64)
        steps[:len(lens)] = lens + m
        lstm_ctx = self.cnn_feat_ctx.is_cuda and isinstance(self.v_net, RNN)
        self._ragged = _hip_lstm.ragged_order(steps, device, T=self.cnn_feat_ctx.shape[0]) if lstm_ctx else None
        self._buckets = None
        n_ep = len(ends)
        if _FWD_BUCKETS > 1 and n_ep >= 4 * _FWD_BUCKETS and self.v_net_type == "lstm":
            order = np.argsort(-lens, kind="stable")
            rank = np.empty(n_ep, np.int64)
            rank[order] = np.arange(n_ep)
            idx_s = np.arange(n)
            idx_s[:covered] = rank[ep_of] * max_len + (np.arange(covered) - np.repeat(starts, lens))
            self._gather_sorted = torch.as_tensor(idx_s, dtype=torch.long, device=device)
            self._ctx_sorted = self.cnn_feat_ctx.index_select(1, torch.as_tensor(order, device=device))
            cuts = [n_ep * k // _FWD_BUCKETS for k in range(_FWD_BUCKETS + 1)]
            lens_sorted = lens[order]
            self._buckets = [(cuts[k], cuts[k + 1], int(m + lens_sorted[cuts[k]])) for k in range(_FWD_BUCKETS)]

    _TRAIN_CONTEXT = ("indices", "cnn_feat_ctx", "gather_indices", "_gather_tm", "_gather_unique", "_ctx_key", "_ragged",
                      "_buckets", "_gather_sorted", "_ctx_sorted", "_frames")

    def adopt_train_context(self, other, x):
        alike = (isinstance(other, VideoStateNet) and self.mode == "train" and other.mode == "train" and other.cnn_feat_ctx is not None
                 and other._ctx_key is not None and self.v_margin == other.v_margin and self.cnn_feat_dim == other.cnn_feat_dim
                 and self.v_net_type == other.v_net_type and self._cnn_table is not None and other._cnn_table is not None
                 and self._cnn_table[0].data_ptr() == other._cnn_table[0].data_ptr()
                 and np.array_equal(self._take_offset_host, other._take_offset_host) and other.cnn_feat_ctx.dtype == x[0].dtype)
        if not alike:
            return self.initialize(x)
        for k in self._TRAIN_CONTEXT:
            if hasattr(other, k):
                setattr(self, k, getattr(other, k))

    def _bucketed_context(self):
        ctx, rnn = self._ctx_sorted, self.v_net
        T, B, _ = ctx.shape
        Hd = rnn.rnn_f.hidden_size
        out_f = ctx.new_zeros(T, B, Hd)
        for i0, i1, Tb in self._buckets:
            Tb = min(Tb, T)
            out_f[:Tb, i0:i1] = rnn._sweep(rnn.rnn_f, ctx[:Tb, i0:i1], False)
        if not rnn.bi_dir:
            return out_f
        return torch.cat((out_f, rnn._sweep(rnn.rnn_b, ctx, True)), 2)

    def forward(self, x, lazy_width=0):
        if self.mode == "test":
            out = torch.cat((self.v_out[[self.t], :], x), dim=1)
            self.t += 1
            return out
        m = self.v_margin
        def tagged(out):
            if not x.requires_grad:
                out._egp_ctx_cols = self.v_hdim
            return out
        if self._buckets is not None:
            ctx = self._bucketed_context()[m:-m].transpose(0, 1).reshape(-1, self.v_hdim)
            return tagged(torch.cat((ctx.index_select(0, self._gather_sorted), x), dim=1))
        ctx = None
        if self._v_ctx is not None:
            (ctx, with_grad), self._v_ctx = self._v_ctx, None
            if with_grad != torch.is_grad_enabled():
                ctx = None
        if ctx is None and isinstance(self.v_net, RNN):
            self.v_net.ragged = self._ragged
            try:
                ctx = self.forward_v_net(self.cnn_feat_ctx)
            finally:
                self.v_net.ragged = None
        elif ctx is None:
            ctx = self.forward_v_net(self.cnn_feat_ctx)
        ctx2d = ctx.reshape(-1, self.v_hdim)
        if self._gather_unique and _gemm.gather_concat_available(ctx2d, self._gather_tm, x):
            if lazy_width and _gemm.fused_gather_available(self.v_hdim, lazy_width, x.shape[1]):
                return _gemm.GatheredInput(ctx2d, self._gather_tm, x)
            return tagged(_gemm.GatherConcat.apply(ctx2d, self._gather_tm, x))
        return tagged(torch.cat((ctx2d.index_select(0, self._gather_tm), x), dim=1))


class Bf16Shadow:

    def __init__(self, master):
        import copy
        self.master = master
        self.shadow = copy.deepcopy(master)
        for name, m in list(master.named_modules()):
            if isinstance(m, nn.modules.batchnorm._BatchNorm):
                parent = self.shadow
                *path, leaf = name.split(".")
                for part in path:
                    parent = getattr(parent, part)
                setattr(parent, leaf, m)
        mp = dict(master.named_parameters())
        self.pairs = []
        for n, p in self.shadow.named_parameters():
            if p is not mp[n]:
                p.data = p.data.to(torch.bfloat16)
                self.pairs.append((mp[n], p))

    @torch.no_grad()
    def pull(self):
        torch._foreach_copy_([s for _, s in self.pairs], [m for m, _ in self.pairs])

    @torch.no_grad()
    def push_grads(self):
        dst, src = [], []
        for m, s in self.pairs:
            if s.grad is None:
                continue
            if m.grad is None:
                m.grad = torch.empty_like(m)
            dst.append(m.grad)
            src.append(s.grad)
        if dst:
            torch._foreach_copy_(dst, src)
        for _, s in self.pairs:
            s.grad = None

    def __call__(self, x):
        return self.shadow(x.to(torch.bfloat16)).float()


class VideoRegNet(nn.Module):

    def __init__(self, out_dim, v_hdim, cnn_fdim, no_cnn=True, frame_shape=(3, 224, 224), mlp_dim=(300, 200),
                 cnn_type="resnet", v_net_type="lstm", v_net_param=None, causal=False):
        super().__init__()
        if not no_cnn and cnn_type != "resnet":
            raise NotImplementedError("only the 'resnet' image encoder is implemented (mobile net is out of scope)")
        self.out_dim, self.cnn_fdim, self.v_hdim, self.no_cnn = out_dim, cnn_fdim, v_hdim, no_cnn
        self.frame_shape = tuple(frame_shape)
        self.cnn = None if no_cnn else ResNet(cnn_fdim)
        self.v_net_type = v_net_type
        self.v_net = _video_net(cnn_fdim, v_hdim, v_net_type, v_net_param, causal)
        self.mlp = MLP(v_hdim, mlp_dim, "relu")
        self.linear = nn.Linear(self.mlp.out_dim, out_dim)

    def forward_v_net(self, x):
        return _run_video_net(self.v_net, x)

    def channels_last(self):
        if self.cnn is not None:
            self.cnn.to(memory_format=torch.channels_last)
            self._nhwc = True
        return self

    def bf16_encoder(self, on=True):
        self.__dict__["_enc16"] = Bf16Shadow(self.cnn) if (on and self.cnn is not None) else None
        return self

    def encoder_grads_ready(self):
        if self.__dict__.get("_enc16") is not None:
            self._enc16.push_grads()

    def encoder_stepped(self):
        if self.__dict__.get("_enc16") is not None:
            self._enc16.pull()

    def _encode(self, frames):
        enc = self.__dict__.get("_enc16")
        if enc is not None and self.training and torch.is_grad_enabled():
            enc.shadow.train(True)
            return enc(frames)
        return self.cnn(frames)

    def _frames(self, x):
        x = x.reshape((-1,) + self.frame_shape)
        return x.contiguous(memory_format=torch.channels_last) if getattr(self, "_nhwc", False) else x

    def forward(self, x):
        if self.cnn is not None:
            x = self._encode(self._frames(x)).view(-1, x.size(1), self.cnn_fdim)
        x = self.forward_v_net(x).reshape(-1, self.v_hdim)
        return self.linear(self.mlp(x))

    def get_cnn_feature(self, x):
        return self._encode(self._frames(x))


class VideoForecastNet(nn.Module):

    def __init__(self, cnn_feat_dim, state_dim, v_hdim=128, v_margin=10, v_net_type="lstm", v_net_param=None,
                 s_hdim=None, s_net_type="id", dynamic_v=False):
        super().__init__()
        if s_net_type not in ("id", "lstm"):
            raise ValueError("s_net_type must be 'id' or 'lstm'")
        s_hdim = state_dim if s_hdim is None else s_hdim
        self.cnn_feat_dim, self.state_dim, self.v_hdim, self.v_margin = cnn_feat_dim, state_dim, v_hdim, v_margin
        self.v_net_type, self.s_net_type, self.s_hdim, self.dynamic_v = v_net_type, s_net_type, s_hdim, dynamic_v
        self.out_dim = v_hdim + s_hdim
        self.v_net = _video_net(cnn_feat_dim, v_hdim, v_net_type, v_net_param, True)
        if s_net_type == "lstm":
            self.s_net = RNN(state_dim, s_hdim, s_net_type, bi_dir=False)
        self.v_out = None
        self.t = 0
        self.indices = self.gather_indices = self.cnn_feat_ctx = None
        self.num_episode = self.max_episode_len = None
        self._cnn_table = None
        self._grp = self._ctx_key = None
        self.set_mode("test")

    def set_mode(self, mode):
        self.mode = mode
        if self.s_net_type == "lstm":
            self.s_net.set_mode("batch" if mode == "train" else "step")

    def forward_v_net(self, x):
        return _run_video_net(self.v_net, x)

    def attach_feature_table(self, table, take_offset):
        host = np.asarray(take_offset, dtype=np.int64)
        cur = getattr(self, "_cnn_table", None)
        if cur is not None and cur[0] is table and np.array_equal(getattr(self, "_take_offset_host", None), host):
            return
        self._cnn_table = (table, torch.as_tensor(host, dtype=torch.long, device=table.device))
        self._take_offset_host = host.copy()
        self._take_len = _take_lengths(take_offset, table.shape[0])

    def check_windows(self, expert_ind, start_ind, length=0):
        _check_windows(self._take_len, expert_ind, start_ind, self.v_margin, length)

    def window_features(self, expert_ind, start_ind, length=0):
        table, off = self._cnn_table
        base = off[expert_ind.long()] + start_ind.long() - self.v_margin
        rows = base.unsqueeze(0) + torch.arange(self.v_margin + length, device=table.device).unsqueeze(1)
        return table[rows]

    def context(self, window):
        return self.forward_v_net(window[:self.v_margin])[-1]

    def s_step(self, state, hc):
        if self.s_net_type != "lstm":
            return state, hc
        h, c = self.s_net.rnn_f(state, hc)
        return h, (h, c)

    def initialize(self, x):
        if self.mode == "test":
            p = next(self.parameters())
            x = x.to(device=p.device, dtype=p.dtype)
            self.v_out = self.context(x.unsqueeze(1) if x.dim() == 2 else x)
            if self.s_net_type == "lstm":
                self.s_net.initialize(self.v_out.shape[0])
            self.t = 0
            return
        masks, cnn_feat, v_metas = x
        device, dtype = masks.device, masks.dtype
        m = self.v_margin
        ends = torch.nonzero(masks == 0).flatten().cpu().numpy()
        n = masks.shape[0]
        starts = np.concatenate(([0], ends[:-1] + 1))
        lens = ends - starts + 1
        max_len = _dist.global_max(int(lens.max()), device)
        self.num_episode, self.max_episode_len = len(ends), max_len
        idx = np.arange(n)
        covered = int(ends[-1]) + 1
        idx[:covered] = np.repeat(np.arange(len(ends)), lens) * max_len + (np.arange(covered) - np.repeat(starts, lens))
        self.indices = idx
        meta = np.asarray(v_metas)[ends]
        T_ctx = m + max_len if self.dynamic_v else m
        if self._cnn_table is not None and self._cnn_table[0].device == device:
            pad = _tuning.pad_to(len(ends), _tuning.EPISODE_BUCKET) if _tuning.enabled() and len(ends) >= 4 * _tuning.EPISODE_BUCKET else 0
            if pad:
                meta = np.concatenate((meta, np.repeat(meta[:1], pad, axis=0)), 0)
                self.num_episode = meta.shape[0]
            self.check_windows(meta[:, 0], meta[:, 1])
            win = self.window_features(torch.as_tensor(meta[:, 0], device=device), torch.as_tensor(meta[:, 1], device=device)).to(dtype)
            ctx = win.new_zeros(T_ctx, meta.shape[0], self.cnn_feat_dim)
            ctx[:m] = win
        else:
            ctx = np.zeros((T_ctx, len(ends), self.cnn_feat_dim))
            for e, (ei, si) in enumerate(meta):
                ctx[:m, e, :] = cnn_feat[int(ei)][int(si) - m: int(si)]
            ctx = torch.as_tensor(ctx, dtype=dtype, device=device)
        self.cnn_feat_ctx = ctx
        self.gather_indices = torch.as_tensor(idx, dtype=torch.long, device=device)
        self._ctx_key = (int(max_len), meta.shape[0], hash(meta.tobytes()))
        self._grp = None

    def state_sequences(self, x):
        s_ctx = x.new_zeros(self.num_episode * self.max_episode_len, self.state_dim)
        s_ctx = s_ctx.index_copy(0, self.gather_indices, x)
        return s_ctx.view(self.num_episode, self.max_episode_len, self.state_dim).transpose(0, 1).contiguous()

    def forward(self, x):
        if self.mode == "test":
            if self.s_net_type == "lstm":
                x = self.s_net(x)
            self.t += 1
            return torch.cat((self.v_out, x), dim=1)
        v_seq = s_seq = None
        if self._grp is not None:
            (v_seq, s_seq, x_ref, with_grad), self._grp = self._grp, None
            if x_ref is not x or with_grad != torch.is_grad_enabled():
                v_seq = s_seq = None
        if v_seq is None:
            v_seq = self.forward_v_net(self.cnn_feat_ctx)
        v_ctx = v_seq[self.v_margin:] if self.dynamic_v else v_seq[[-1]].expand(self.max_episode_len, -1, -1)
        v_out = v_ctx.transpose(0, 1).reshape(-1, self.v_hdim).index_select(0, self.gather_indices)
        if self.s_net_type == "lstm":
            if s_seq is None:
                s_seq = self.s_net(self.state_sequences(x))
            s_out = s_seq.transpose(0, 1).reshape(-1, self.s_hdim).index_select(0, self.gather_indices)
        else:
            s_out = x
        return torch.cat((v_out, s_out), dim=1)


def grouped_video_context(nets):
    if _LSTM_IMPL == "torch" or len(nets) < 1:
        return False
    n0 = nets[0]
    for n in nets:
        if not (isinstance(n, VideoStateNet) and n.mode == "train" and n._buckets is None and getattr(n.v_net, "cell_type", None) == "lstm"
                and n.cnn_feat_ctx is not None and n.cnn_feat_ctx.shape == n0.cnn_feat_ctx.shape and n._ctx_key == n0._ctx_key
                and n.cnn_feat_ctx.dtype == n0.cnn_feat_ctx.dtype and n.v_net.bi_dir == n0.v_net.bi_dir):
            return False
    cells, revs = [], []
    for n in nets:
        cells.append(n.v_net.rnn_f); revs.append(False)
        if n.v_net.bi_dir:
            cells.append(n.v_net.rnn_b); revs.append(True)
    x = n0.cnn_feat_ctx
    if not _hip_lstm.group_available(x, cells):
        return False
    hs = _hip_lstm.lstm_group(x, cells, revs, pairs=n0.v_net.bi_dir, ragged=n0._ragged,
                              frames=getattr(n0, "_frames", None))
    for i, n in enumerate(nets):
        n._v_ctx = (hs[i], torch.is_grad_enabled())
    return True


def grouped_forecast_context(nets, x):
    if _LSTM_IMPL == "torch" or len(nets) < 2 or x is None:
        return False
    n0 = nets[0]
    for n in nets:
        if not (isinstance(n, VideoForecastNet) and n.mode == "train" and n.s_net_type == "lstm" and n.cnn_feat_ctx is not None
                and n._ctx_key is not None and n._ctx_key == n0._ctx_key and n.cnn_feat_ctx.shape == n0.cnn_feat_ctx.shape
                and n.cnn_feat_ctx.dtype == n0.cnn_feat_ctx.dtype and n.dynamic_v == n0.dynamic_v and n.state_dim == n0.state_dim
                and isinstance(n.v_net, RNN) and not n.v_net.bi_dir and not n.s_net.bi_dir and n.v_net.cell_type == "lstm" and n.s_net.cell_type == "lstm"):
            return False
    v_cells, s_cells = [n.v_net.rnn_f for n in nets], [n.s_net.rnn_f for n in nets]
    s_in = n0.state_sequences(x)
    if not (_hip_lstm.group_available(n0.cnn_feat_ctx, v_cells) and _hip_lstm.group_available(s_in, s_cells)):
        return False
    fwd = [False] * len(nets)
    hv = _hip_lstm.lstm_group(n0.cnn_feat_ctx, v_cells, fwd)
    hs = _hip_lstm.lstm_group(s_in, s_cells, fwd)
    for n, a, b in zip(nets, hv, hs):
        n._grp = (a, b, x, torch.is_grad_enabled())
    return True


class _BasicBlock(nn.Module):
    def __init__(self, cin, cout, stride):
        super().__init__()
        self.conv1 = nn.Conv2d(cin, cout, 3, stride, 1, bias=False)
        self.bn1 = nn.BatchNorm2d(cout)
        self.conv2 = nn.Conv2d(cout, cout, 3, 1, 1, bias=False)
        self.bn2 = nn.BatchNorm2d(cout)
        self.downsample = None
        if stride != 1 or cin != cout:
            self.downsample = nn.Sequential(nn.Conv2d(cin, cout, 1, stride, bias=False), nn.BatchNorm2d(cout))

    def forward(self, x):
        idt = x if self.downsample is None else self.downsample(x)
        out = torch.relu(self.bn1(self.conv1(x)))
        out = self.bn2(self.conv2(out))
        return torch.relu(out + idt)


class ResNet18(nn.Module):

    def __init__(self, out_dim):
        super().__init__()
        self.out_dim = out_dim
        self.conv1 = nn.Conv2d(3, 64, 7, 2, 3, bias=False)
        self.bn1 = nn.BatchNorm2d(64)
        self.maxpool = nn.MaxPool2d(3, 2, 1)
        chans, layers, cin = (64, 128, 256, 512), [], 64
        for i, c in enumerate(chans):
            layers.append(nn.Sequential(_BasicBlock(cin, c, 1 if i == 0 else 2), _BasicBlock(c, c, 1)))
            cin = c
        self.layer1, self.layer2, self.layer3, self.layer4 = layers
        self.avgpool = nn.AdaptiveAvgPool2d(1)
        self.fc = nn.Linear(512, out_dim)

    def forward(self, x):
        x = self.maxpool(torch.relu(self.bn1(self.conv1(x))))
        x = self.layer4(self.layer3(self.layer2(self.layer1(x))))
        return self.fc(torch.flatten(self.avgpool(x), 1))


class ResNet(nn.Module):

    def __init__(self, out_dim, fix_params=False):
        super().__init__()
        self.out_dim = out_dim
        self.resnet = ResNet18(out_dim)
        if fix_params:
            for name, p in self.resnet.named_parameters():
                p.requires_grad = name.startswith("fc.")

    def forward(self, x):
        return self.resnet(x)
```

include/egopose_hip.h:

```cpp
#ifndef EGOPOSE_HIP_H
#define EGOPOSE_HIP_H

#include <stdint.h>

#ifdef __cplusplus
extern "C" {
#endif

#define EGP_OK 0
#define EGP_E_INVALID (-1)
#define EGP_E_HIP (-2)
#define EGP_E_STATE (-3)
#define EGP_E_PHYSICS (-4)

#define EGP_MAX_NV 64
#define EGP_MAX_BODY 32
#define EGP_EXPERT_ROW 168

typedef struct egp_ctx egp_ctx;
typedef struct egp_physics egp_physics;
typedef struct egp_engine egp_engine;

typedef struct egp_model_desc {
    int32_t nq, nv, nu, nbody, nM;
    const int32_t *body_qpos_start;
    const int32_t *body_ndof;
    const int32_t *dof_parentid;
    const int32_t *dof_Madr;
    const int32_t *ee_body;
    const double *jkp, *jkd, *a_ref, *a_scale, *torque_lim;
    const double *b_diffw;
    double sub_dt;
    int32_t frame_skip;
    int32_t episode_len;
    double w_p, w_v, w_e, w_rp, w_rv;
    double k_p, k_v, k_e, k_rh, k_rq, k_rl, k_ra;
    double v_ord;
    int32_t decay;
    int32_t obs_heading;
    int32_t obs_keep_root_heading;
    int32_t obs_coord_root;
    int32_t obs_vel;
    int32_t action_torque;
    int32_t obs_phase;
} egp_model_desc;
int32_t egp_obs_dim(const egp_ctx *ctx);

typedef struct egp_expert_table {
    int32_t n_takes;
    int32_t n_frames;
    const int32_t *take_offset;
    const double *qpos;
    const double *qvel;
    const double *rlinv_local;
    const double *rangv;
    const double *rq_rmh;
    const double *ee_pos;
    const double *bquat;
    const double *bangvel;
    const double *head_height_lb;
} egp_expert_table;

const char *egp_last_error(void);
const char *egp_version(void);
int64_t egp_abi_sizeof(const char *name);

int egp_create(const egp_model_desc *desc, int device, egp_ctx **out);
int egp_destroy(egp_ctx *ctx);
int egp_set_reward_weights(egp_ctx *ctx, const egp_model_desc *desc);
int egp_set_pd_variant(egp_ctx *ctx, int variant);
int egp_upload_experts(egp_ctx *ctx, const egp_expert_table *tbl);


enum {
    EGP_QUAT_MUL = 0, EGP_QUAT_INV = 1, EGP_QUAT_FROM_EULER_SXYZ = 2, EGP_QUAT_HEADING_Q = 3, EGP_QUAT_DE_HEADING = 4,
    EGP_QUAT_TRANSFORM_VEC_ROOT = 5, EGP_QUAT_TRANSFORM_VEC_HEADING = 6, EGP_QUAT_ROTATION = 7, EGP_QUAT_DIFF_HALF_ANGLE = 8,
    EGP_QUAT_N_OPS = 9
};
int egp_quat_op_f64(int32_t op, const double *a, const double *b, int32_t n, double *out, void *stream);
int egp_quat_op_f32(int32_t op, const float *a, const float *b, int32_t n, float *out, void *stream);

int egp_body_quat_f64(egp_ctx *ctx, const double *qpos, int32_t n, double *bquat, void *stream);
int egp_body_quat_f32(egp_ctx *ctx, const float *qpos, int32_t n, float *bquat, void *stream);

int egp_obs_f64(egp_ctx *ctx, const double *qpos, const double *qvel, const int32_t *phase_t, int32_t n, double *obs, void *stream);
int egp_obs_f32(egp_ctx *ctx, const float *qpos, const float *qvel, const int32_t *phase_t, int32_t n, float *obs, void *stream);

int egp_pd_torque_f64(egp_ctx *ctx, const double *qpos, const double *qvel, const double *action,
                      const double *qM, const double *qfrc_bias, int32_t n,
                      double *torque, double *torque_raw, void *stream);
int egp_pd_torque_f32(egp_ctx *ctx, const float *qpos, const float *qvel, const float *action,
                      const float *qM, const float *qfrc_bias, int32_t n,
                      float *torque, float *torque_raw, void *stream);

int egp_reward_quat_v3_f64(egp_ctx *ctx, const double *cur_qpos, const double *prev_qpos,
                           const double *ee_wpos, const int32_t *t, const int32_t *frame,
                           const int32_t *end, const int32_t *active, double end_reward, int32_t n,
                           double *reward, double *c_info, void *stream);
int egp_reward_quat_v3_f32(egp_ctx *ctx, const float *cur_qpos, const float *prev_qpos,
                           const float *ee_wpos, const int32_t *t, const int32_t *frame,
                           const int32_t *end, const int32_t *active, double end_reward, int32_t n,
                           float *reward, float *c_info, void *stream);
#define EGP_REWARD_CONSTANT 1
#define EGP_REWARD_POSE_DIST 2
int egp_reward_simple_f64(egp_ctx *ctx, int32_t kind, const double *qpos, const int32_t *frame, const int32_t *end, const int32_t *active,
                          double end_reward, int32_t n, double *reward, double *cinfo, void *stream);

int egp_pose_features_f64(egp_ctx *ctx, const double *cur_qpos, const double *prev_qpos, const double *ee_wpos,
                          int32_t n, int32_t expert_convention, double *qvel, double *rlinv_local, double *rangv,
                          double *rq_rmh, double *ee_pos, double *bquat, double *bangvel, void *stream);
int egp_pose_features_f32(egp_ctx *ctx, const float *cur_qpos, const float *prev_qpos, const float *ee_wpos,
                          int32_t n, int32_t expert_convention, float *qvel, float *rlinv_local, float *rangv,
                          float *rq_rmh, float *ee_pos, float *bquat, float *bangvel, void *stream);

int64_t egp_zfilter_workspace_bytes(int32_t n, int32_t dim);
int egp_zfilter_f64(const double *x, const int32_t *active, int32_t n, int32_t dim,
                    const double *state_in, double *state_out, int32_t update, double clip,
                    double *y, void *workspace, void *stream);
int egp_zfilter_f32(const float *x, const int32_t *active, int32_t n, int32_t dim,
                    const double *state_in, double *state_out, int32_t update, double clip,
                    float *y, void *workspace, void *stream);

int egp_obs_zfilter_f64(egp_ctx *ctx, const double *qpos, const double *qvel, const int32_t *phase_t, const int32_t *active, int32_t n,
                        const double *state_in, double *state_out, double clip, double *y, double *y2,
                        int32_t write_only_active, void *workspace, void *stream);
int egp_obs_zfilter_f32(egp_ctx *ctx, const float *qpos, const float *qvel, const int32_t *phase_t, const int32_t *active, int32_t n,
                        const double *state_in, double *state_out, double clip, float *y, float *y2,
                        int32_t write_only_active, void *workspace, void *stream);
int32_t egp_obs_zfilter_split_max_rows(void);
int egp_obs_zfilter_stats_f64(egp_ctx *ctx, const double *qpos, const double *qvel, const int32_t *phase_t, const int32_t *active, int32_t n, void *workspace,
                              void *stream);
int egp_obs_zfilter_apply_f64(egp_ctx *ctx, const double *qpos, const double *qvel, const int32_t *phase_t, int32_t n, const double *state_in, double *state_out,
                              double clip, double *y, double *y2, void *workspace, void *stream);

int64_t egp_gae_workspace_bytes(int32_t n);
int egp_gae_f64(const double *rewards, const double *masks, const double *values, int32_t n,
                double gamma, double tau, double *adv_raw, double *returns, double *stats,
                void *workspace, void *stream);
int egp_gae_f32(const float *rewards, const float *masks, const float *values, int32_t n,
                double gamma, double tau, float *adv_raw, float *returns, double *stats,
                void *workspace, void *stream);
int egp_gae_standardize_f64(double *adv, int32_t n, const double *stats, void *stream);
int egp_gae_standardize_f32(float *adv, int32_t n, const double *stats, void *stream);


typedef struct egp_gemm_desc {
    int32_t M, N, K;
    const float *A; int64_t lda; int32_t a_kcontig;
    const float *B; int64_t ldb; int32_t b_kcontig;
    float *C; int64_t ldc;
    const float *bias; int32_t relu;
    const float *mask; int64_t ldmask;
    int32_t terms, splits, accumulate;
    float *bias_grad;
    float *workspace;
    const int64_t *a_rows; const float *A2; int64_t lda2; int32_t a_split; int64_t a_src_rows;
    const int64_t *b_krows; const float *B2; int64_t ldb2; int32_t b_split; int64_t b_src_rows;
    const int64_t *c_rows;
    const int64_t *a_krows;
} egp_gemm_desc;
typedef struct egp_ppo_loss_desc {
    int32_t n, n_pol, act_dim;
    const int64_t *rows;
    const float *pred; const float *returns;
    const float *mean; int64_t ld_mean;
    const float *actions; int64_t ld_act;
    const float *log_std;
    const float *adv;
    float *fixed_logp; int32_t write_fixed;
    double clip_eps, inv_n_val, inv_n_exp;
    float *d_pred;
    float *d_mean; int64_t ld_dmean;
    float *d_log_std;
    double *losses;
    void *workspace;
} egp_ppo_loss_desc;
int64_t egp_ppo_loss_workspace_bytes(int32_t n, int32_t n_pol, int32_t act_dim);
int egp_ppo_loss_f32(const egp_ppo_loss_desc *desc, void *stream);

struct egp_minibatch_plan_desc {
    int32_t n, state_dim, act_dim, batch;
    const int64_t *perm;
    const float *states; int64_t ld_states;
    const float *actions; int64_t ld_act;
    const float *returns; const float *adv; const float *fixed_logp; const float *exps;
    float *out_states; float *out_actions; float *out_returns; float *out_adv; float *out_fixed_logp; float *out_exps;
    int32_t *mb_n_exp;
};
typedef struct egp_minibatch_plan_desc egp_minibatch_plan_desc;
int egp_minibatch_plan_f32(const egp_minibatch_plan_desc *desc, void *stream);

#define EGP_PPO_LOSS_MB_MAX_ROWS 16384
struct egp_ppo_loss_mb_desc {
    int32_t n, act_dim;
    const float *pred; const float *returns;
    const float *mean; int64_t ld_mean;
    const float *actions; int64_t ld_act;
    const float *log_std;
    const float *adv; const float *fixed_logp; const float *exps;
    const int32_t *n_exp;
    double clip_eps;
    float *d_pred;
    float *d_mean; int64_t ld_dmean;
    float *d_log_std;
    double *losses;
};
typedef struct egp_ppo_loss_mb_desc egp_ppo_loss_mb_desc;
int egp_ppo_loss_mb_f32(const egp_ppo_loss_mb_desc *desc, void *stream);

typedef struct egp_adam_segment {
    int64_t begin, end;
    double lr, beta1, beta2, eps, weight_decay, bias1, bias2, max_norm;
    int32_t clip_group;
} egp_adam_segment;
#define EGP_ADAM_MAX_SEGMENTS 8
int64_t egp_adam_workspace_bytes(void);
int egp_adam_step_f32(int32_t n_seg, const egp_adam_segment *seg, const float *grad, float *param, float *exp_avg, float *exp_avg_sq,
                      void *workspace, double *norms_out, void *stream);
int egp_adam_step_f64(int32_t n_seg, const egp_adam_segment *seg, const float *grad, double *param, double *exp_avg, double *exp_avg_sq,
                      float *shadow, void *workspace, double *norms_out, void *stream);
int egp_adam_step_f64g(int32_t n_seg, const egp_adam_segment *seg, const double *grad, double *param, double *exp_avg, double *exp_avg_sq,
                       void *workspace, double *norms_out, void *stream);

int egp_gather_concat_f32(const float *ctx, int64_t ld_ctx, const int64_t *idx, const float *x, int64_t ldx, int32_t n, int32_t H, int32_t S,
                          float *out, int64_t ldo, void *stream);
int egp_scatter_rows_f32(const float *dout, int64_t ldd, const int64_t *idx, int32_t n, int32_t H, float *dctx, int64_t ld_ctx, void *stream);
int64_t egp_gemm_workspace_floats(int32_t M, int32_t N, int32_t ones_col, int32_t splits);
int egp_gemm_f32(const egp_gemm_desc *desc, void *stream);

struct egp_tcn_desc {
    int32_t T, B, C_in, C_out, taps, shift0, dshift;
    const float *X; int64_t ldx;
    const float *W;
    const float *bias; int32_t relu;
    const float *mask; int64_t ldmask;
    const float *gate; int64_t ldgate;
    const float *X2; int64_t ldx2; int32_t C2; const float *W2; const float *b2; int32_t x2_after_act;
    float *out; int64_t ldout;
    float *out2; int64_t ldout2;
};
typedef struct egp_tcn_desc egp_tcn_desc;
int egp_tcn_conv_f32(const egp_tcn_desc *desc, void *stream);

#define EGP_LSTM_GATES_TORCH 0
#define EGP_LSTM_GATES_UNIT_MAJOR 1
int32_t egp_lstm_gate_layout(void);
int egp_lstm_fwd_f32(const float *gates_x, const float *w_hh, int32_t T, int32_t B, int32_t hidden, int32_t reverse,
                     float *h_out, float *gates_save, float *cells_save, void *stream);
int egp_lstm_bwd_f32(const float *dh_out, const float *gates_save, const float *cells_save, const float *w_hh,
                     int32_t T, int32_t B, int32_t hidden, int32_t reverse, float *d_pre, void *stream);
int egp_lstm_group_fwd_f32(const float *gates_x, const float *w_hh, int32_t T, int32_t B, int32_t hidden, int32_t n_problems,
                           int32_t reverse_mask, float *const *h_out, int32_t ld_h, float *gates_save, float *cells_save, void *stream);
int egp_lstm_group_bwd_f32(const float *const *dh_out, int32_t ld_dh, const float *gates_save, const float *cells_save, const float *w_hh,
                           int32_t T, int32_t B, int32_t hidden, int32_t n_problems, int32_t reverse_mask, float *d_pre, float *d_bias,
                           void *stream);

int egp_lstm_group_fwd_len_f32(const float *gates_x, const float *w_hh, int32_t T, int32_t B, int32_t hidden, int32_t n_problems,
                               int32_t reverse_mask, float *const *h_out, int32_t ld_h, float *gates_save, float *cells_save,
                               const int32_t *seq_order, const int32_t *seq_steps, int32_t leave_skipped, const int32_t *seq_base,
                               void *stream);
int egp_lstm_group_bwd_len_f32(const float *const *dh_out, int32_t ld_dh, const float *gates_save, const float *cells_save, const float *w_hh,
                               int32_t T, int32_t B, int32_t hidden, int32_t n_problems, int32_t reverse_mask, float *d_pre, float *d_bias,
                               const int32_t *seq_order, const int32_t *seq_steps, int32_t leave_skipped, void *stream);
int egp_lstm_group_bwd_rows_f32(const float *const *dh_out, int32_t ld_dh, const float *gates_save, const float *cells_save, const float *w_hh,
                                int32_t T, int32_t B, int32_t hidden, int32_t n_problems, int32_t reverse_mask, float *d_pre, float *d_bias_rows,
                                const int32_t *seq_order, const int32_t *seq_steps, int32_t leave_skipped, void *stream);

typedef struct egp_dynamics_desc {
    int32_t nbody, njoint;
    const int32_t *body_parent;
    const double *body_pos;
    const double *body_com;
    const double *body_inertia;
    const double *body_mass;
    const int32_t *body_ndof;
    const double *joint_axis;
    const double *joint_anchor;
    double armature;
    double gravity[3];
} egp_dynamics_desc;
int egp_set_dynamics_model(egp_ctx *ctx, const egp_dynamics_desc *desc);
int egp_dynamics_f64(egp_ctx *ctx, const double *qpos, const double *qvel, int32_t n, double *qM, int64_t ld_m,
                     double *qfrc_bias, double *xpos, void *stream);

#define EGP_POSE2D_NKP 12
int egp_set_pose2d_bodies(egp_ctx *ctx, const int32_t *kp_body , const int32_t *roles );
int egp_pose2d_f64(egp_ctx *ctx, const double *qpos , const double *gt ,
                   const int32_t *flip , double *p_out , double *dist ,
                   int32_t *valid , int64_t n, void *stream);


typedef struct egp_mlp_layer {
    const float *wt;
    const float *bias;
    int32_t in_dim, out_dim;
} egp_mlp_layer;
int64_t egp_mlp_pack_floats(int32_t in_dim, int32_t out_dim);
int egp_mlp_pack_f32(const float *weight, int64_t ldw, int32_t in_dim, int32_t out_dim, float *packed, void *stream);
int egp_policy_gaussian_f32(const float *ctx_rows, int64_t ctx_row_stride, int32_t ctx_dim, const int64_t *t_idx,
                            const double *state, int32_t state_dim, int32_t n, const egp_mlp_layer *layers,
                            int32_t n_layers, int32_t activation, const float *log_std, const float *noise,
                            double *action, float *mean_out, void *stream);
int egp_policy_gaussian_staged_f32(const float *ctx_rows, int64_t ctx_row_stride, int32_t ctx_dim, const int64_t *t_idx,
                                   const double *state, int32_t state_dim, int32_t n, const egp_mlp_layer *layers,
                                   int32_t n_layers, int32_t activation, const float *log_std, const float *noise,
                                   double *action, float *mean_out, const void *stage_src, void *stage_dst, int64_t stage_bytes,
                                   void *stream);
int egp_policy_gaussian_filter_f32(egp_ctx *ctx, const float *ctx_rows, int64_t ctx_row_stride, int32_t ctx_dim, const int64_t *t_idx,
                                   const double *qpos, const double *qvel, const int32_t *phase_t, int32_t n, const double *zf_in, double *zf_out,
                                   double clip, double *y, double *y2, const void *zf_workspace,
                                   const egp_mlp_layer *layers, int32_t n_layers, int32_t activation, const float *log_std,
                                   const float *noise, double *action, float *mean_out, const void *stage_src, void *stage_dst,
                                   int64_t stage_bytes, void *stream);
int egp_policy_value_filter_f32(egp_ctx *ctx, const float *ctx_rows, int64_t ctx_row_stride, int32_t ctx_dim, const float *vctx_rows,
                                int64_t vctx_row_stride, int32_t vctx_dim, const int64_t *t_idx, const double *qpos, const double *qvel,
                                const int32_t *phase_t, int32_t n, const double *zf_in, double *zf_out, double clip, double *y, double *y2,
                                const egp_mlp_layer *layers, int32_t n_layers, int32_t activation, const float *log_std,
                                const float *noise, double *action, float *mean_out, const egp_mlp_layer *vlayers, int32_t n_vlayers,
                                int32_t vactivation, float *value_out, void *stream);
int egp_policy_forecast_f32(const float *ctx_rows, int64_t ctx_row_stride, int32_t ctx_dim, const int64_t *t_idx,
                            const double *state, int32_t state_dim, const egp_mlp_layer *cell, float *h, float *c,
                            int64_t hc_row_stride, int32_t n, const egp_mlp_layer *layers, int32_t n_layers, int32_t activation,
                            const float *log_std, const float *noise, double *action, float *mean_out, void *stream);
int egp_policy_forecast_filter_f32(egp_ctx *ctx, const float *ctx_rows, int64_t ctx_row_stride, int32_t ctx_dim, const int64_t *t_idx,
                                   const double *qpos, const double *qvel, const int32_t *phase_t, int32_t n,
                                   const double *zf_in, double *zf_out, double clip, double *y, double *y2, const void *zf_workspace,
                                   const egp_mlp_layer *cell, float *h, float *c, int64_t hc_row_stride,
                                   const egp_mlp_layer *layers, int32_t n_layers, int32_t activation, const float *log_std,
                                   const float *noise, double *action, float *mean_out, void *stream);

typedef struct egp_physics_vtable {
    void *user;
    int (*reset)(void *user, int32_t env, const double *qpos, const double *qvel);
    int (*step)(void *user, int32_t env, const double *ctrl);
    int (*drain)(void *user, int32_t env, double *qpos, double *qvel, double *qM, double *qfrc_bias,
                 double *xpos);
    void (*destroy)(void *user);
    const char *name;
    int64_t (*inertia_epoch)(void *user, int32_t env);
} egp_physics_vtable;

int egp_physics_register(const egp_physics_vtable *vt, int32_t n_env, egp_physics **out);
typedef struct egp_surrogate_desc {
    int32_t nq, nv, nu, nbody, nM, njoint;
    const double *qM0;
    const double *Minv0;
    const int32_t *body_parent;
    const double *body_pos;
    const int32_t *body_ndof;
    const double *joint_axis;
    const double *joint_anchor;
    double sub_dt;
    double damping;
    double support_k, support_c;
} egp_surrogate_desc;
int egp_physics_create_surrogate(const egp_surrogate_desc *desc, int32_t n_env, egp_physics **out);
int egp_physics_destroy(egp_physics *p);
const char *egp_physics_name(const egp_physics *p);
int egp_physics_reset_host(egp_physics *p, int32_t env, const double *qpos_host, const double *qvel_host);
int egp_physics_step_host(egp_physics *p, int32_t env, const double *ctrl_host);
int egp_physics_drain_host(egp_physics *p, int32_t env, double *qpos_host, double *qvel_host,
                           double *qM_host, double *qfrc_bias_host, double *xpos_host);

typedef struct egp_engine_desc {
    int32_t n_env;
    int32_t n_threads;
    int32_t n_groups;
    int32_t device_dynamics;
} egp_engine_desc;

int egp_engine_create(egp_ctx *ctx, egp_physics *phys, const egp_engine_desc *desc, egp_engine **out);
int egp_engine_destroy(egp_engine *e);
int egp_engine_state(egp_engine *e, double **qpos, double **qvel, double **ee_wpos, double **head_z_host,
                     double **qpos_host, double **qvel_host, double **prev_qpos);
int egp_engine_reset(egp_engine *e, const int32_t *env_ids_host, int32_t n, const double *qpos_host,
                     const double *qvel_host, void *stream);
int egp_engine_step_async(egp_engine *e, int32_t group, const double *action, const int32_t *active_host,
                          void *ready_event);
int egp_engine_wait(egp_engine *e, int32_t group, void *stream);
int egp_engine_timing(egp_engine *e, double *phys_s, double *gpu_wait_s, double *k1_ms_events, int64_t *k1_launches);
int egp_engine_reset_timing(egp_engine *e);
int64_t egp_engine_k1_env_substeps(egp_engine *e);
int64_t egp_engine_inertia_uploads(egp_engine *e);
double egp_engine_event_overhead_ms(egp_engine *e);
int egp_engine_set_profile(egp_engine *e, int on);
int egp_engine_layout(egp_engine *e, int32_t *pack_ld, int32_t *n_env, int32_t *n_threads, int32_t *n_groups);
int egp_engine_group_range(egp_engine *e, int32_t group, int32_t *env_begin, int32_t *env_end);
typedef struct egp_rollout_tick {
    egp_ctx *ctx; egp_engine *eng; void *stream;
    int32_t n_env, nmax, obs_dim, nu, nq, nv, ctx_dim, ctx_T, episode_len, reward_job, has_fix_head_lb;
    double end_reward, zf_clip, fix_head_lb;
    int64_t *cur_t, *frame_base, *e_ind, *s_ind, *steps_done;
    uint8_t *active; int32_t *active_i32;
    const double *head_z, *head_lb;
    uint8_t *rec_valid, *rec_done; int64_t *rec_e_ind, *rec_s_ind;
    double *states, *next_states, *actions, *rewards, *cinfo;
    const float *noise;
    const float *v_out; int64_t v_stride;
    const egp_mlp_layer *layers; int32_t n_layers, activation; const float *log_std;
    uint8_t *slab_host, *slab_dev;
    const double *qpos, *qvel, *prev_qpos, *ee;
    void *zf_workspace;
    int32_t *reset_scratch;
    int32_t defer_apply;
} egp_rollout_tick;
int egp_rollout_tick_pre(const egp_rollout_tick *d, int32_t group, int32_t a, int32_t b, int32_t k, void *ready_event,
                         int32_t apply_pending, const double *zf_cur, double *zf_new);
int egp_rollout_tick_apply(const egp_rollout_tick *d, int32_t group, int32_t a, int32_t b, int32_t k, const double *zf_cur, double *zf_new);
int egp_rollout_tick_post(const egp_rollout_tick *d, int32_t group, int32_t a, int32_t b, int32_t k, const double *zf_cur, double *zf_new,
                          int32_t *n_done, double *wait_s);
int egp_rollout_reset(const egp_rollout_tick *d, int32_t group, int32_t a, int32_t b, int32_t k, const int32_t *ids, int32_t n,
                      const int64_t *e_ind, const int64_t *s_ind, const int64_t *frame_rows, const int64_t *cur_t0, const double *qpos, const double *qvel,
                      const float *ctx_rows, const double *zf_cur, double *zf_new);
void *egp_engine_group_stream(egp_engine *e, int32_t group);

int egp_engine_set_reward_job(egp_engine *e, int32_t group, const int32_t *t, const int32_t *frame, const int32_t *end,
                              const int32_t *active, double end_reward, double *reward, double *cinfo);
int egp_debug_burn(int64_t us, int32_t blocks, float *sink, void *stream);
int egp_engine_substeps_per_launch(egp_engine *e);
int32_t egp_engine_envs_per_wave(egp_engine *e, int32_t *resident_capacity);
int32_t egp_engine_go_words_in_vram(egp_engine *e);
int egp_engine_server_trace(egp_engine *e, int32_t group, int64_t *device_ticks, double *host_us);
typedef struct egp_host_probe_result {
    double pcie_read_gbps, pcie_read_us_per_pass;
    double go_rtt_us_p50, go_rtt_us_p99, go_rtt_us_max;
    double spin_gap_us_max, spin_gap_us_median_of_thread_max, spin_lost_frac;
    int32_t pcie_read_rows, go_rtt_n, go_in_vram, large_bar, spin_threads, spin_gaps_over_5us;
} egp_host_probe_result;
int egp_host_probe(int32_t device, int32_t n_threads, int32_t millis, egp_host_probe_result *out);
int32_t egp_device_usable_cus(int32_t device);
int32_t egp_physics_n_env(const egp_physics *p);

#ifdef __cplusplus
}
#endif
#endif
```

Baseline: 1.001 million.

## Sum LSTM input gradients per shared frame and mask out-of-range output grads

Adds a kernel that gathers d_pre rows from overlapping sequence windows into one row per unique frame. The input-weight gradient then becomes a GEMM over the frame table rather than over all T*B window rows, cutting GEMM size when windows overlap heavily. It also passes per-sequence output ranges into the backward LSTM kernel so dh outside the valid output window reads from a zero row. That lets the context gradient buffer be allocated with empty instead of zeros. The cost is an extra reduction kernel, host-side index building, and more plumbing through the autograd functions.

After: 994,300 (median of 2 runs). No clear change (-0.6%).

```diff
diff --git a/egopose_amd/_lib.py b/egopose_amd/_lib.py
--- a/egopose_amd/_lib.py
+++ b/egopose_amd/_lib.py
@@ -242,6 +242,8 @@
     "egp_lstm_group_fwd_len_f32": (C.c_int, [vp, vp, _i32, _i32, _i32, _i32, _i32, C.POINTER(C.c_void_p), _i32, vp, vp, vp, vp, _i32, vp, vp]),
     "egp_lstm_group_bwd_len_f32": (C.c_int, [C.POINTER(C.c_void_p), _i32, vp, vp, vp, _i32, _i32, _i32, _i32, _i32, vp, vp, vp, vp, _i32, vp]),
     "egp_lstm_group_bwd_rows_f32": (C.c_int, [C.POINTER(C.c_void_p), _i32, vp, vp, vp, _i32, _i32, _i32, _i32, _i32, vp, vp, vp, vp, _i32, vp]),
+    "egp_lstm_group_bwd_range_f32": (C.c_int, [C.POINTER(C.c_void_p), _i32, vp, vp, vp, _i32, _i32, _i32, _i32, _i32, vp, vp, vp, vp, _i32, vp, vp, vp]),
+    "egp_lstm_dpre_frames_f32": (C.c_int, [vp, _i32, _i32, _i32, _i32, vp, vp, vp, vp, vp, _i32, vp, vp]),
     "egp_set_dynamics_model": (C.c_int, [vp, C.POINTER(DynamicsDesc)]),
     "egp_dynamics_f64": (C.c_int, [vp, vp, vp, _i32, vp, C.c_int64, vp, vp, vp]),
     "egp_set_pose2d_bodies": (C.c_int, [vp, c_int_p, c_int_p]),
diff --git a/egopose_amd/csrc/egp_lstm.hip b/egopose_amd/csrc/egp_lstm.hip
--- a/egopose_amd/csrc/egp_lstm.hip
+++ b/egopose_amd/csrc/egp_lstm.hip
@@ -40,7 +40,11 @@
     const int *steps;
     int leave_skipped;
     const int *seq_base;
+    const int *out_lo;
+    const int *out_hi;
 };
+
+__device__ float g_lstm_zero_row[128];
 
 template <int ROWS>
 __device__ __forceinline__ int lstm_group_steps(const LstmGroup &grp, int reverse, int r0, int B, int T) {
@@ -226,7 +230,7 @@
     f32x4 pg[PD][NP];
     float pc[PD][NP], pdh[PD][NP];
     bool live[NP];
-    int rowc[NP];
+    int rowc[NP], olo[NP], ohi[NP];
 #pragma unroll
     for (int qq = 0; qq < NP; ++qq) {
         dc_next[qq] = 0.f; dh_rec[qq] = 0.f; dsum[qq] = f32x4{0.f, 0.f, 0.f, 0.f};
@@ -234,6 +238,8 @@
         live[qq] = FULL || r0 + r < B;
         const int pos = live[qq] ? r0 + r : B - 1;
         rowc[qq] = grp.order ? grp.order[pos] : pos;
+        olo[qq] = grp.out_lo ? grp.out_lo[rowc[qq]] : 0;
+        ohi[qq] = grp.out_lo ? grp.out_hi[rowc[qq]] : T;
     }
     const int Tp = lstm_group_steps<ROWS>(grp, reverse, r0, B, T);
     const int Tz = grp.leave_skipped ? lstm_group_steps<8>(grp, reverse, r0 & ~7, B, T) : T;
@@ -252,7 +258,8 @@
             const long row = (long)f_t * B + rowc[qq];                                               \
             pg[D][qq] = ld_save(reinterpret_cast<const f32x4 *>(gates + row * ld + 4 * j));         \
             pc[D][qq] = ld_save(cells + row * LH + j);                                               \
-            pdh[D][qq] = dh_out[row * ld_dh + j];                                                    \
+            const bool f_in = f_t >= olo[qq] && f_t < ohi[qq];                                       \
+            pdh[D][qq] = *(f_in ? dh_out + row * ld_dh + j : g_lstm_zero_row + j);                   \
         }                                                                                            \
     }
 
@@ -359,6 +366,33 @@
     }
 }
 
+template <int U>
+__global__ __launch_bounds__(512) void k_lstm_dpre_frames(const float *__restrict__ dpre, int T, int B, int ld, int n_fwd_cols,
+                                                          const int *__restrict__ seq_base, const int *__restrict__ t_lim,
+                                                          const int *__restrict__ sorted, const int *__restrict__ lo,
+                                                          const int *__restrict__ hi, float *__restrict__ g_out) {
+    const int f = (int)blockIdx.x, c = 4 * (int)threadIdx.x;
+    const bool fwd_col = c < n_fwd_cols;
+    const int i0 = max(lo[f], 0), i1 = min(hi[f], B);
+    f32x4 acc = f32x4{0.f, 0.f, 0.f, 0.f};
+    for (int i = i0; i < i1; i += U) {
+        f32x4 v[U];
+        bool ok[U];
+#pragma unroll
+        for (int k = 0; k < U; ++k) {
+            const int b = min(max(sorted[min(i + k, i1 - 1)], 0), B - 1);
+            const int t = f - seq_base[b];
+            const int lim = t_lim ? min(t_lim[b], T) : T;
+            ok[k] = i + k < i1 && t >= 0 && t < (fwd_col ? lim : T);
+            const long row = ok[k] ? (long)t * B + b : 0;
+            v[k] = *reinterpret_cast<const f32x4 *>(dpre + row * ld + c);
+        }
+#pragma unroll
+        for (int k = 0; k < U; ++k) acc += ok[k] ? v[k] : f32x4{0.f, 0.f, 0.f, 0.f};
+    }
+    *reinterpret_cast<f32x4 *>(g_out + (long)f * ld + c) = acc;
+}
+
 }
 
 using namespace egp;
@@ -410,8 +444,10 @@
 
 static int lstm_group_bwd(const float *const *dh_out, int32_t ld_dh, const float *gates_save, const float *cells_save, const float *w_hh,
                           int32_t T, int32_t B, int32_t hidden, int32_t n_problems, int32_t reverse_mask, float *d_pre, float *d_bias,
-                          int db_rows, const int32_t *seq_order, const int32_t *seq_steps, int32_t leave_skipped, void *stream) {
+                          int db_rows, const int32_t *seq_order, const int32_t *seq_steps, int32_t leave_skipped, void *stream,
+                          const int32_t *out_lo = nullptr, const int32_t *out_hi = nullptr) {
     EGP_REQUIRE((seq_order == nullptr) == (seq_steps == nullptr), "seq_order and seq_steps go together");
+    EGP_REQUIRE((out_lo == nullptr) == (out_hi == nullptr), "out_lo and out_hi go together");
     EGP_REQUIRE(hidden == 64 || hidden == 128, "egp_lstm kernels are built for hidden size 64 and 128");
     EGP_REQUIRE(n_problems >= 1 && n_problems <= 4, "1..4 problems per group");
     EGP_REQUIRE(T >= 0 && B >= 0, "negative size");
@@ -423,7 +459,7 @@
         EGP_REQUIRE(dh_out[p], "NULL d h_out");
         g.dh[p] = dh_out[p];
     }
-    g.order = seq_order; g.steps = seq_steps; g.leave_skipped = seq_steps && leave_skipped;
+    g.order = seq_order; g.steps = seq_steps; g.leave_skipped = seq_steps && leave_skipped; g.out_lo = out_lo; g.out_hi = out_hi;
     launch_bwd_mfma(hidden, n_problems, gates_save, cells_save, w_hh, T, B, g, d_pre, (hipStream_t)stream);
     return lstm_launch_check("k_lstm_bwd_mfma (group)");
 }
@@ -514,4 +550,33 @@
                           seq_steps, leave_skipped, stream);
 }
 
-}
+int egp_lstm_group_bwd_range_f32(const float *const *dh_out, int32_t ld_dh, const float *gates_save, const float *cells_save, const float *w_hh,
+                                 int32_t T, int32_t B, int32_t hidden, int32_t n_problems, int32_t reverse_mask, float *d_pre, float *d_bias_rows,
+                                 const int32_t *seq_order, const int32_t *seq_steps, int32_t leave_skipped, const int32_t *out_lo,
+                                 const int32_t *out_hi, void *stream) {
+    EGP_REQUIRE(d_bias_rows, "NULL d_bias_rows");
+    if (T == 0) return egp_lstm_group_bwd_rows_f32(dh_out, ld_dh, gates_save, cells_save, w_hh, T, B, hidden, n_problems, reverse_mask, d_pre,
+                                                   d_bias_rows, seq_order, seq_steps, leave_skipped, stream);
+    return lstm_group_bwd(dh_out, ld_dh, gates_save, cells_save, w_hh, T, B, hidden, n_problems, reverse_mask, d_pre, d_bias_rows, 1, seq_order,
+                          seq_steps, leave_skipped, stream, out_lo, out_hi);
+}
+
+int egp_lstm_dpre_frames_f32(const float *d_pre, int32_t T, int32_t B, int32_t n_cols, int32_t n_fwd_cols, const int32_t *seq_base,
+                             const int32_t *t_lim, const int32_t *sorted, const int32_t *lo, const int32_t *hi, int32_t n_frames,
+                             float *g_out, void *stream) {
+    EGP_REQUIRE(T >= 0 && B >= 0 && n_frames >= 0, "negative size");
+    EGP_REQUIRE(n_cols >= 4 && n_cols % 4 == 0 && n_cols <= 2048, "n_cols: a multiple of 4 up to 2048 (four problems of hidden size 128)");
+    EGP_REQUIRE(n_fwd_cols >= 0 && n_fwd_cols <= n_cols && n_fwd_cols % 4 == 0, "n_fwd_cols: a multiple of 4 within n_cols");
+    if (n_frames == 0) return EGP_OK;
+    EGP_REQUIRE(g_out, "NULL g_out");
+    if (T == 0 || B == 0) {
+        EGP_HIP_CHECK(hipMemsetAsync(g_out, 0, sizeof(float) * (size_t)n_frames * n_cols, (hipStream_t)stream));
+        return EGP_OK;
+    }
+    EGP_REQUIRE(d_pre && seq_base && sorted && lo && hi, "NULL pointer");
+    k_lstm_dpre_frames<8><<<dim3(n_frames), dim3(n_cols / 4), 0, (hipStream_t)stream>>>(d_pre, T, B, n_cols, n_fwd_cols, seq_base, t_lim, sorted,
+                                                                                       lo, hi, g_out);
+    return lstm_launch_check("k_lstm_dpre_frames");
+}
+
+}
diff --git a/egopose_amd/gemm.py b/egopose_amd/gemm.py
--- a/egopose_amd/gemm.py
+++ b/egopose_amd/gemm.py
@@ -221,8 +221,8 @@
 
 class GatheredInput:
 
-    def __init__(self, ctx2d, idx, x):
-        self.ctx2d, self.idx, self.x = ctx2d, idx, x
+    def __init__(self, ctx2d, idx, x, ranged=False):
+        self.ctx2d, self.idx, self.x, self.ranged = ctx2d, idx, x, bool(ranged)
         self.shape = (x.shape[0], ctx2d.shape[1] + x.shape[1])
         self.dtype, self.device, self.is_cuda = x.dtype, x.device, x.is_cuda
 
@@ -255,7 +255,7 @@
 class GatherMlpHead(torch.autograd.Function):
 
     @staticmethod
-    def forward(ctx, ctx2d, idx, x, *params):
+    def forward(ctx, ctx2d, idx, x, ranged, *params):
         Ws, bs = params[0::2], params[1::2]
         ctx2d, x = ctx2d.contiguous(), (x if x.stride(1) == 1 else x.contiguous())
         h = gemm(ctx2d, Ws[0].contiguous(), True, True, bias=bs[0], relu=len(Ws) > 1, a_rows=idx, a2=x)
@@ -263,7 +263,7 @@
         for i in range(1, len(Ws)):
             hs.append(linear_fwd(hs[-1], Ws[i].contiguous(), bs[i], relu=i < len(Ws) - 1))
         ctx.save_for_backward(ctx2d, idx, x, *hs[:-1], *Ws)
-        ctx.n_layers = len(Ws)
+        ctx.n_layers, ctx.ranged = len(Ws), bool(ranged)
         return hs[-1]
 
     @staticmethod
@@ -274,28 +274,28 @@
         dz = dout.contiguous()
         grads = [None] * (2 * nl)
         for i in range(nl - 1, 0, -1):
-            need_w, need_b = ctx.needs_input_grad[3 + 2 * i], ctx.needs_input_grad[4 + 2 * i]
+            need_w, need_b = ctx.needs_input_grad[4 + 2 * i], ctx.needs_input_grad[5 + 2 * i]
             if need_w or need_b:
                 dW, db = linear_wgrad(dz, hs[i - 1], want_bias=True)
                 grads[2 * i], grads[2 * i + 1] = (dW if need_w else None), (db if need_b else None)
             dz = linear_dgrad(dz, Ws[i].contiguous(), mask=hs[i - 1])
         H, S = ctx2d.shape[1], x.shape[1]
-        if ctx.needs_input_grad[3] or ctx.needs_input_grad[4]:
+        if ctx.needs_input_grad[4] or ctx.needs_input_grad[5]:
             n = dz.shape[0]
             dW, db = gemm(dz, ctx2d, False, False, splits=pick_splits(dz.shape[1], H + S + 1, n), want_bias_grad=True, b_krows=idx, b2=x)
-            grads[0], grads[1] = (dW if ctx.needs_input_grad[3] else None), (db if ctx.needs_input_grad[4] else None)
+            grads[0], grads[1] = (dW if ctx.needs_input_grad[4] else None), (db if ctx.needs_input_grad[5] else None)
         dctx = None
         if ctx.needs_input_grad[0]:
-            dctx = torch.zeros_like(ctx2d)
+            dctx = torch.empty_like(ctx2d) if ctx.ranged else torch.zeros_like(ctx2d)
             gemm(dz, Ws[0][:, :H], True, False, out=dctx, c_rows=idx)
-        return (dctx, None, None, *grads)
+        return (dctx, None, None, None, *grads)
 
 
 def gather_mlp_head(gi, layers, head):
     params = []
     for l in list(layers) + [head]:
         params += [l.weight, l.bias]
-    return GatherMlpHead.apply(gi.ctx2d, gi.idx, gi.x, *params)
+    return GatherMlpHead.apply(gi.ctx2d, gi.idx, gi.x, gi.ranged, *params)
 
 
 class GatherConcat(torch.autograd.Function):
diff --git a/egopose_amd/lstm.py b/egopose_amd/lstm.py
--- a/egopose_amd/lstm.py
+++ b/egopose_amd/lstm.py
@@ -10,6 +10,9 @@
 from . import gemm as G
 
 HIDDEN_SIZES = (64, 128)
+FRAME_WGRAD = True
+ROWS_MIN = 4096
+_DPRE_HOOK = None
 
 
 def available(x, cell):
@@ -114,7 +117,7 @@
 class LstmGroup(torch.autograd.Function):
 
     @staticmethod
-    def forward(ctx, x, reverse_mask, P, width, train, ragged, frames, *params):
+    def forward(ctx, x, reverse_mask, P, width, train, ragged, frames, out_range, *params):
         lib = L.load()
         T, B, D = x.shape
         w_ih, w_hh, b_ih, b_hh = params[0::4], params[1::4], params[2::4], params[3::4]
@@ -129,11 +132,12 @@
         bias = (torch.cat([b_ih[p] for p in pord]) + torch.cat([b_hh[p] for p in pord])).index_select(0, bperm)
         rows = None
         if ragged is not None and ragged.rows is not None and 0 < nf and G.enabled() and G.fused_rows_available() \
-                and ragged.T == T and ragged.rows.shape[0] >= 4096 and D >= 32:
+                and ragged.T == T and ragged.rows.shape[0] >= ROWS_MIN and D >= 32:
             rows = ragged.rows
-        seq_base, gates_buf = None, None
+        seq_base, gates_buf, table, fidx = None, None, None, None
         if frames is not None and G.enabled():
-            table, seq_base = frames
+            table, seq_base = frames[:2]
+            fidx = frames[2] if len(frames) > 2 and FRAME_WGRAD else None
             gx = G.linear_fwd(table, w_in, bias)
             gates_buf = torch.empty(T * B, P * 4 * H, dtype=x.dtype, device=x.device) if train else None
         elif rows is not None:
@@ -161,8 +165,10 @@
                                                _p(gates), _p(cells), _p(order), _p(steps), leave, _p(seq_base), _s()), "egp_lstm_group_fwd_len_f32")
         outs = tuple(h_buf[i, 1:T + 1] for i in range(n_out))
         if train:
-            ctx.save_for_backward(x2, w_in, w_hh_all, h_buf, gates, cells)
+            ctx.save_for_backward(table if fidx is not None else x2, w_in, w_hh_all, h_buf, gates, cells)
             ctx.meta = (T, B, D, H, P, width, reverse_mask)
+            ctx.fidx, ctx.seq_base = fidx, (seq_base if fidx is not None else None)
+            ctx.out_range = out_range
             ctx.ragged, ctx.rows, ctx.pord, ctx.nf, ctx.kmask, ctx.leave = ragged, rows, pord, nf, kmask, leave
         return outs
 
@@ -181,13 +187,27 @@
         db_rows = torch.empty(P, B, 4 * H, dtype=x2.dtype, device=x2.device)
         order, steps = (ragged.order, ragged.steps) if ragged is not None else (None, None)
         leave = int(bool(ctx.leave) and not ctx.needs_input_grad[0])
-        L.check(lib.egp_lstm_group_bwd_rows_f32(ptrs, W, _p(gates), _p(cells), _p(w_hh_all), T, B, H, P, kmask, _p(dpre), _p(db_rows),
-                                                _p(order), _p(steps), leave, _s()), "egp_lstm_group_bwd_rows_f32")
+        if ctx.out_range is not None:
+            o_lo, o_hi = ctx.out_range
+            L.check(lib.egp_lstm_group_bwd_range_f32(ptrs, W, _p(gates), _p(cells), _p(w_hh_all), T, B, H, P, kmask, _p(dpre), _p(db_rows),
+                                                     _p(order), _p(steps), leave, _p(o_lo), _p(o_hi), _s()), "egp_lstm_group_bwd_range_f32")
+        else:
+            L.check(lib.egp_lstm_group_bwd_rows_f32(ptrs, W, _p(gates), _p(cells), _p(w_hh_all), T, B, H, P, kmask, _p(dpre), _p(db_rows),
+                                                    _p(order), _p(steps), leave, _s()), "egp_lstm_group_bwd_rows_f32")
+        if _DPRE_HOOK is not None:
+            _DPRE_HOOK(dpre, ctx)
         db = db_rows.sum(1)
         d3 = dpre.view(T, B, P * 4 * H)
         use_g = G.enabled()
         nfc = nf * 4 * H
-        if rows is not None:
+        if ctx.fidx is not None:
+            fidx, n_frames = ctx.fidx, x2.shape[0]
+            t_lim = ragged.t_lim if rows is not None else None
+            gsum = torch.empty(n_frames, P * 4 * H, dtype=x2.dtype, device=x2.device)
+            L.check(lib.egp_lstm_dpre_frames_f32(_p(dpre), T, B, P * 4 * H, nfc, _p(ctx.seq_base), _p(t_lim), _p(fidx.sorted), _p(fidx.lo),
+                                                 _p(fidx.hi), n_frames, _p(gsum), _s()), "egp_lstm_dpre_frames_f32")
+            dw_ih_all = G.linear_wgrad(gsum, x2, want_bias=False)
+        elif rows is not None:
             n_rows = rows.shape[0]
             parts = [G.gemm(dpre[:, :nfc], x2, False, False, splits=G.pick_splits(nfc, D, n_rows), a_krows=rows, b_krows=rows)]
             if nf < P:
@@ -217,7 +237,7 @@
             d_b = db_t[q]
             grads[4 * p:4 * p + 4] = [dw_ih, dw_hh, d_b, d_b]
         d_x = dpre.mm(w_in).view(T, B, D) if ctx.needs_input_grad[0] else None
-        return (d_x, None, None, None, None, None, None, *grads)
+        return (d_x, None, None, None, None, None, None, None, *grads)
 
 
 def _wants_grad(x, params):
@@ -233,8 +253,9 @@
 
 class Ragged:
 
-    def __init__(self, order, steps, rows, n_seq, T):
+    def __init__(self, order, steps, rows, n_seq, T, t_lim=None):
         self.order, self.steps, self.rows, self.n_seq, self.T = order, steps, rows, n_seq, T
+        self.t_lim = t_lim
 
 
 def ragged_order(seq_steps, device, T=None):
@@ -242,7 +263,7 @@
     B = st.shape[0]
     order = np.argsort(-st, kind="stable")
     st_sorted = st[order]
-    rows = None
+    rows = t_lim = None
     if T is not None and B > 0:
         wg = np.maximum.reduceat(st_sorted, np.arange(0, B, 8))
         t_wg = np.minimum(np.repeat(wg, 8)[:B], int(T))
@@ -252,22 +273,49 @@
             t_seq[order] = t_wg
             stepped = np.arange(int(T), dtype=np.int64)[:, None] < t_seq[None, :]
             rows = torch.as_tensor(np.flatnonzero(stepped), dtype=torch.int64, device=device)
+            t_lim = torch.as_tensor(t_seq.astype(np.int32), device=device)
     return Ragged(torch.as_tensor(order, dtype=torch.int32, device=device), torch.as_tensor(st_sorted, dtype=torch.int32, device=device),
-                  rows, B, T)
-
-
-def lstm_group(x, cells, reverses, pairs=False, ragged=None, frames=None):
+                  rows, B, T, t_lim)
+
+
+def frame_index_arrays(base, T, n_frames):
+    base = np.asarray(base, dtype=np.int64).reshape(-1)
+    if base.size and (base.min() < 0 or base.max() + int(T) > int(n_frames)):
+        raise ValueError("windows must lie inside the table: 0 <= base and base + T <= n_frames")
+    srt = np.argsort(base, kind="stable")
+    f = np.arange(int(n_frames), dtype=np.int64)
+    lo = np.searchsorted(base[srt], f - int(T), side="right")
+    hi = np.searchsorted(base[srt], f, side="right")
+    return srt.astype(np.int32), lo.astype(np.int32), hi.astype(np.int32)
+
+
+class FrameIndex:
+
+    def __init__(self, base, T, n_frames, device):
+        srt, lo, hi = frame_index_arrays(base, T, n_frames)
+        self.T, self.n_frames, self.n_seq = int(T), int(n_frames), srt.shape[0]
+        self.sorted, self.lo, self.hi = (torch.as_tensor(a, device=device) for a in (srt, lo, hi))
+
+
+def lstm_group(x, cells, reverses, pairs=False, ragged=None, frames=None, out_range=None):
     mask = sum(1 << i for i, r in enumerate(reverses) if r)
     params = [t for c in cells for t in (c.weight_ih, c.weight_hh, c.bias_ih, c.bias_hh)]
     if ragged is not None and ragged.n_seq != x.shape[1]:
         ragged = None
     if frames is not None:
-        table, base = frames
+        table, base = frames[:2]
         ok = (table.is_cuda and table.dtype == x.dtype and table.dim() == 2 and table.shape[1] == x.shape[2] and table.is_contiguous()
               and base.dtype == torch.int32 and base.is_cuda and base.is_contiguous() and base.shape[0] == x.shape[1] and not x.requires_grad)
         if not ok:
             frames = None
-    return list(LstmGroup.apply(x.contiguous(), mask, len(cells), 2 if pairs else 1, _wants_grad(x, params), ragged, frames, *params))
+        elif len(frames) > 2 and not (isinstance(frames[2], FrameIndex) and frames[2].T == x.shape[0] and frames[2].n_seq == x.shape[1]
+                                      and frames[2].n_frames == table.shape[0] and x.shape[0] > 0 and 4 * len(cells) * cells[0].hidden_size <= 2048):
+            frames = frames[:2]
+    if out_range is not None:
+        lo, hi = out_range
+        if not all(t.is_cuda and t.dtype == torch.int32 and t.is_contiguous() and t.shape == (x.shape[1],) for t in (lo, hi)):
+            raise ValueError("out_range: two contiguous int32 device tensors of B entries")
+    return list(LstmGroup.apply(x.contiguous(), mask, len(cells), 2 if pairs else 1, _wants_grad(x, params), ragged, frames, out_range, *params))
 
 
 def lstm_direction(cell, x, reverse):
diff --git a/egopose_amd/nets.py b/egopose_amd/nets.py
--- a/egopose_amd/nets.py
+++ b/egopose_amd/nets.py
@@ -16,6 +16,7 @@
 from .tcn import TemporalConvNet
 
 _FWD_BUCKETS = 1
+OUT_RANGE = True
 _LSTM_IMPL = os.environ.get("EGP_LSTM", "hip")
 
 _ACT = {"tanh": torch.tanh, "relu": torch.relu, "sigmoid": torch.sigmoid}
@@ -284,6 +285,7 @@
         self.cnn_feat_ctx = None
         self._buckets = None
         self._v_ctx = None
+        self._out_range = None
         self._ctx_key = None
         self._cnn_table = None
         self._ragged = None
@@ -326,6 +328,7 @@
         masks, cnn_feat, v_metas = x
         device, dtype = masks.device, masks.dtype
         self._frames = None
+        self._out_range = None
         ends = torch.nonzero(masks == 0).flatten().cpu().numpy()
         n = masks.shape[0]
         starts = np.concatenate(([0], ends[:-1] + 1))
@@ -349,7 +352,8 @@
             n_rows = self.cnn_feat_ctx.shape[0] * self.cnn_feat_ctx.shape[1]
             if table.dtype == dtype and table.is_contiguous() and 2 * table.shape[0] <= n_rows:
                 base = self._take_offset_host[meta[:, 0].astype(np.int64)] + meta[:, 1].astype(np.int64) - m
-                self._frames = (table, torch.as_tensor(base.astype(np.int32), device=device))
+                self._frames = (table, torch.as_tensor(base.astype(np.int32), device=device),
+                                _hip_lstm.FrameIndex(base, self.cnn_feat_ctx.shape[0], table.shape[0], device))
         else:
             ctx = np.zeros((max_len + 2 * m, len(ends), self.cnn_feat_dim))
             for e, (ei, si) in enumerate(meta):
@@ -362,6 +366,10 @@
         self._ctx_key = (int(max_len), meta.shape[0], hash(meta.tobytes()))
         steps = np.zeros(self.cnn_feat_ctx.shape[1], np.int64)
         steps[:len(lens)] = lens + m
+        if OUT_RANGE and covered == n and self.cnn_feat_ctx.is_cuda:
+            o_lo = np.zeros(steps.shape[0], np.int32)
+            o_lo[:len(lens)] = m
+            self._out_range = (torch.as_tensor(o_lo, device=device), torch.as_tensor(steps.astype(np.int32), device=device))
         lstm_ctx = self.cnn_feat_ctx.is_cuda and isinstance(self.v_net, RNN)
         self._ragged = _hip_lstm.ragged_order(steps, device, T=self.cnn_feat_ctx.shape[0]) if lstm_ctx else None
         self._buckets = None
@@ -379,7 +387,7 @@
             self._buckets = [(cuts[k], cuts[k + 1], int(m + lens_sorted[cuts[k]])) for k in range(_FWD_BUCKETS)]
 
     _TRAIN_CONTEXT = ("indices", "cnn_feat_ctx", "gather_indices", "_gather_tm", "_gather_unique", "_ctx_key", "_ragged",
-                      "_buckets", "_gather_sorted", "_ctx_sorted", "_frames")
+                      "_buckets", "_gather_sorted", "_ctx_sorted", "_frames", "_out_range")
 
     def adopt_train_context(self, other, x):
         alike = (isinstance(other, VideoStateNet) and self.mode == "train" and other.mode == "train" and other.cnn_feat_ctx is not None
@@ -418,11 +426,11 @@
         if self._buckets is not None:
             ctx = self._bucketed_context()[m:-m].transpose(0, 1).reshape(-1, self.v_hdim)
             return tagged(torch.cat((ctx.index_select(0, self._gather_sorted), x), dim=1))
-        ctx = None
+        ctx, ranged = None, False
         if self._v_ctx is not None:
-            (ctx, with_grad), self._v_ctx = self._v_ctx, None
+            (ctx, with_grad, ranged), self._v_ctx = self._v_ctx, None
             if with_grad != torch.is_grad_enabled():
-                ctx = None
+                ctx, ranged = None, False
         if ctx is None and isinstance(self.v_net, RNN):
             self.v_net.ragged = self._ragged
             try:
@@ -434,7 +442,7 @@
         ctx2d = ctx.reshape(-1, self.v_hdim)
         if self._gather_unique and _gemm.gather_concat_available(ctx2d, self._gather_tm, x):
             if lazy_width and _gemm.fused_gather_available(self.v_hdim, lazy_width, x.shape[1]):
-                return _gemm.GatheredInput(ctx2d, self._gather_tm, x)
+                return _gemm.GatheredInput(ctx2d, self._gather_tm, x, ranged=ranged)
             return tagged(_gemm.GatherConcat.apply(ctx2d, self._gather_tm, x))
         return tagged(torch.cat((ctx2d.index_select(0, self._gather_tm), x), dim=1))
 
@@ -686,9 +694,9 @@
     if not _hip_lstm.group_available(x, cells):
         return False
     hs = _hip_lstm.lstm_group(x, cells, revs, pairs=n0.v_net.bi_dir, ragged=n0._ragged,
-                              frames=getattr(n0, "_frames", None))
+                              frames=getattr(n0, "_frames", None), out_range=getattr(n0, "_out_range", None))
     for i, n in enumerate(nets):
-        n._v_ctx = (hs[i], torch.is_grad_enabled())
+        n._v_ctx = (hs[i], torch.is_grad_enabled(), getattr(n0, "_out_range", None) is not None)
     return True
 
 
diff --git a/include/egopose_hip.h b/include/egopose_hip.h
--- a/include/egopose_hip.h
+++ b/include/egopose_hip.h
@@ -265,6 +265,13 @@
 int egp_lstm_group_bwd_rows_f32(const float *const *dh_out, int32_t ld_dh, const float *gates_save, const float *cells_save, const float *w_hh,
                                 int32_t T, int32_t B, int32_t hidden, int32_t n_problems, int32_t reverse_mask, float *d_pre, float *d_bias_rows,
                                 const int32_t *seq_order, const int32_t *seq_steps, int32_t leave_skipped, void *stream);
+int egp_lstm_group_bwd_range_f32(const float *const *dh_out, int32_t ld_dh, const float *gates_save, const float *cells_save, const float *w_hh,
+                                 int32_t T, int32_t B, int32_t hidden, int32_t n_problems, int32_t reverse_mask, float *d_pre, float *d_bias_rows,
+                                 const int32_t *seq_order, const int32_t *seq_steps, int32_t leave_skipped, const int32_t *out_lo,
+                                 const int32_t *out_hi, void *stream);
+int egp_lstm_dpre_frames_f32(const float *d_pre, int32_t T, int32_t B, int32_t n_cols, int32_t n_fwd_cols, const int32_t *seq_base,
+                             const int32_t *t_lim, const int32_t *sorted, const int32_t *lo, const int32_t *hi, int32_t n_frames,
+                             float *g_out, void *stream);
 
 typedef struct egp_dynamics_desc {
     int32_t nbody, njoint;
```
